# laboroai/border

Measured on AMD Instinct MI355X. Metric: agent opt-steps/sec (DQN Atari 84x84x4, batch 256), higher is better.
Workload: dtype f32 (conv2 / conv3 forward: 3xbf16 operand split, 6 products)

## Files before the change

border_amd/csrc/conv1_dw_bf16.hpp:

```cpp
#pragma once
#include "conv1_bf16.hpp"

namespace bdr {

struct Conv1DwArgs {
    const uint8_t* x;
    const float* dy;
    float* part;
    size_t part_stride;
    int B;
};

constexpr int C1DW_LDM = 408;
constexpr int C1DW_ROW = 88, C1DW_CH = 84 * 88 + 96;
#ifndef C1DW_WAVES_PER_EU
#define C1DW_WAVES_PER_EU 3
#endif
constexpr int C1DW_PF = 2;

struct __attribute__((packed, aligned(4))) U32x4A4 { uint32_t x, y, z, w; };

template <int PH>
__device__ __forceinline__ uint32_t u8pair_to_bf16(uint32_t d0, uint32_t d1)
{
    const uint32_t f0 = __float_as_uint((float)((d0 >> (8 * PH)) & 255u)), f1 = __float_as_uint((float)((d1 >> (8 * PH)) & 255u));
    return __builtin_amdgcn_perm(f1, f0, 0x07060302u);
}

#ifdef C1DW_TRACE
__device__ unsigned long long* g_c1dw_trace;
#define C1DW_TP(slot) do { if (threadIdx.x == 0 && g_c1dw_trace) g_c1dw_trace[blockIdx.x * 4 + (slot)] = wall_clock64(); } while (0)
#else
#define C1DW_TP(slot) do { } while (0)
#endif

__device__ __forceinline__ void c1dw_load_step(const uint8_t* src, int s, int g, U32x4A4 (&d)[2])
{
#pragma unroll
    for (int q = 0; q < 2; ++q) {
        const int quad = 2 * s + q;
        const int oh = quad / 5, ow0 = 4 * (quad - 5 * oh);
        const uint32_t* p = reinterpret_cast<const uint32_t*>(src + (4 * oh) * C1DW_ROW + 4 * ow0);
        d[q].x = p[0]; d[q].y = p[1]; d[q].z = p[2]; d[q].w = p[3];
    }
}

template <int PH, int TPW>
__device__ __forceinline__ void c1dw_steps(const uint8_t* const (&src)[TPW], U32x4A4 (&ring)[TPW][C1DW_PF + 1][2], const uint16_t* planes, int i, int g,
                                           f32x16 (&acc)[TPW])
{
    uint4 bq[3], bn[3];
#pragma unroll
    for (int pl = 0; pl < 3; ++pl) bq[pl] = *reinterpret_cast<const uint4*>(&planes[(pl * 32 + i) * C1DW_LDM + 200 * g]);
#pragma unroll
    for (int s = 0; s < 25; ++s) {
        if (s + 1 < 25) {
#pragma unroll
            for (int pl = 0; pl < 3; ++pl) bn[pl] = *reinterpret_cast<const uint4*>(&planes[(pl * 32 + i) * C1DW_LDM + 8 * (s + 1) + 200 * g]);
        }
#pragma unroll
        for (int t = 0; t < TPW; ++t) {
            U32x4A4 (&cur)[2] = ring[t][s % (C1DW_PF + 1)];
            if (s + C1DW_PF < 25) c1dw_load_step(src[t], s + C1DW_PF, g, ring[t][(s + C1DW_PF) % (C1DW_PF + 1)]);
            uint4 av;
            av.x = u8pair_to_bf16<PH>(cur[0].x, cur[0].y);
            av.y = u8pair_to_bf16<PH>(cur[0].z, cur[0].w);
            av.z = u8pair_to_bf16<PH>(cur[1].x, cur[1].y);
            av.w = u8pair_to_bf16<PH>(cur[1].z, cur[1].w);
            const bf16x8 af = __builtin_bit_cast(bf16x8, av);
#pragma unroll
            for (int pl = 2; pl >= 0; --pl)
                acc[t] = __builtin_amdgcn_mfma_f32_32x32x16_bf16(af, __builtin_bit_cast(bf16x8, bq[pl]), acc[t], 0, 0, 0);
        }
#pragma unroll
        for (int pl = 0; pl < 3; ++pl) bq[pl] = bn[pl];
        __builtin_amdgcn_sched_barrier(0);
    }
}

template <int NS>
static __global__ __launch_bounds__(512) __attribute__((amdgpu_waves_per_eu(NS <= 4 ? C1DW_WAVES_PER_EU : 2, NS <= 4 ? C1DW_WAVES_PER_EU : 2))) void k_conv1_dw_bf16(Conv1DwArgs a)
{
    C1DW_TP(0);
    constexpr int TASKS = 4 * ((NS + 1) / 2), TPW = (TASKS + 7) / 8;
    extern __shared__ __attribute__((aligned(16))) uint8_t c1dw_lds[];
    uint16_t* planes = reinterpret_cast<uint16_t*>(c1dw_lds);
    uint32_t* ximg_l = reinterpret_cast<uint32_t*>(c1dw_lds + 3 * 32 * C1DW_LDM * 2);
    float (*sred)[32] = reinterpret_cast<float (*)[32]>(c1dw_lds + 3 * 32 * C1DW_LDM * 2 + NS * C1DW_CH);
    const int tid = threadIdx.x, lane = tid & 63, wave = __builtin_amdgcn_readfirstlane(tid >> 6);
    const int i = lane & 31, g = lane >> 5;
    const int pn = tid & 31, pmg = tid >> 5;
    const int phase = wave & 3;

    f32x16 acc[TPW];
#pragma unroll
    for (int t = 0; t < TPW; ++t)
#pragma unroll
        for (int r = 0; r < 16; ++r) acc[t][r] = 0.f;
    float bsum = 0.f;

    int c_of[TPW], rowoff; bool live[TPW];
    rowoff = ((i >> 1) & 7) * C1DW_ROW + 4 * (i & 1) + g * (40 * C1DW_ROW);
#pragma unroll
    for (int t = 0; t < TPW; ++t) {
        const int task = wave + 8 * t;
        live[t] = task < TASKS;
        const int c = 2 * ((live[t] ? task : 0) >> 2) + (i >> 4);
        c_of[t] = c < NS ? c : NS - 1;
    }

    for (int img = blockIdx.x; img < a.B; img += gridDim.x) {
        constexpr int XPT = (NS * 441 + 511) / 512;
        uint4 xst[XPT];
        {
            const uint4* xg = reinterpret_cast<const uint4*>(a.x + (size_t)img * (NS * 7056));
#pragma unroll
            for (int k = 0; k < XPT; ++k) { const int t = tid + 512 * k; xst[k] = xg[t < NS * 441 ? t : NS * 441 - 1]; }
        }
        {
            const float* dyb = a.dy + (size_t)img * 400 * 32;
            float s = 0.f;
#pragma unroll
            for (int q0 = 0; q0 < 7; q0 += 4) {
                float y[4][4];
#pragma unroll
                for (int q = 0; q < 4; ++q) {
                    const int quad = pmg + 16 * (q0 + q);
#pragma unroll
                    for (int j = 0; j < 4; ++j) y[q][j] = (q0 + q < 7 && quad < 100) ? dyb[(size_t)(4 * quad + j) * 32 + pn] : 0.f;
                }
#pragma unroll
                for (int q = 0; q < 4; ++q) {
                    const int quad = pmg + 16 * (q0 + q);
                    if (q0 + q < 7 && quad < 100) {
                        uint32_t hi[4], mid[4], lo[4];
#pragma unroll
                        for (int j = 0; j < 4; ++j) {
                            s += y[q][j];
                            hi[j] = __float_as_uint(y[q][j]) & 0xffff0000u;
                            const float r1 = y[q][j] - __uint_as_float(hi[j]);
                            mid[j] = __float_as_uint(r1) & 0xffff0000u;
                            const float r2 = r1 - __uint_as_float(mid[j]);
                            lo[j] = __float_as_uint(r2) & 0xffff0000u;
                        }
                        const int o = pn * C1DW_LDM + 4 * quad;
                        *reinterpret_cast<uint2*>(&planes[0 * 32 * C1DW_LDM + o]) = uint2{(hi[0] >> 16) | hi[1], (hi[2] >> 16) | hi[3]};
                        *reinterpret_cast<uint2*>(&planes[1 * 32 * C1DW_LDM + o]) = uint2{(mid[0] >> 16) | mid[1], (mid[2] >> 16) | mid[3]};
                        *reinterpret_cast<uint2*>(&planes[2 * 32 * C1DW_LDM + o]) = uint2{(lo[0] >> 16) | lo[1], (lo[2] >> 16) | lo[3]};
                    }
                }
            }
            sred[pmg][pn] = s;
        }
#pragma unroll
        for (int k = 0; k < XPT; ++k) {
            const int t = tid + 512 * k;
            if (t < NS * 441) {
                const uint32_t w[4] = {xst[k].x, xst[k].y, xst[k].z, xst[k].w};
#pragma unroll
                for (int e = 0; e < 4; ++e) {
                    const int d = 4 * t + e, c = d / 1764, rem = d - c * 1764, r = rem / 21;
                    ximg_l[c * (C1DW_CH / 4) + r * (C1DW_ROW / 4) + (rem - r * 21)] = w[e];
                }
            }
        }
        __syncthreads();
        C1DW_TP(1);
        if (tid < 32) {
            float t = sred[0][tid];
#pragma unroll
            for (int k = 1; k < 16; ++k) t += sred[k][tid];
            bsum += t;
        }

        const uint8_t* src[TPW];
        U32x4A4 ring[TPW][C1DW_PF + 1][2];
#pragma unroll
        for (int t = 0; t < TPW; ++t) {
            src[t] = reinterpret_cast<const uint8_t*>(ximg_l) + c_of[t] * C1DW_CH + rowoff;
#pragma unroll
            for (int s0 = 0; s0 < C1DW_PF; ++s0) c1dw_load_step(src[t], s0, g, ring[t][s0]);
        }
        if (live[0]) {
            if (phase == 0) c1dw_steps<0, TPW>(src, ring, planes, i, g, acc);
            else if (phase == 1) c1dw_steps<1, TPW>(src, ring, planes, i, g, acc);
            else if (phase == 2) c1dw_steps<2, TPW>(src, ring, planes, i, g, acc);
            else c1dw_steps<3, TPW>(src, ring, planes, i, g, acc);
        }
        C1DW_TP(2);
        __syncthreads();
    }

    float* part = a.part + (size_t)blockIdx.x * a.part_stride;
#pragma unroll
    for (int t = 0; t < TPW; ++t) {
        if (!live[t]) continue;
        const int pair = (wave + 8 * t) >> 2;
#pragma unroll
        for (int r = 0; r < 16; ++r) {
            const int row = (r & 3) + 8 * (r >> 2) + 4 * g;
            const int c = 2 * pair + (row >> 4), kh = (row >> 1) & 7, kw = phase + 4 * (row & 1);
            if (c < NS) part[(size_t)(c * 64 + kh * 8 + kw) * 32 + i] = acc[t][r];
        }
    }
    if (tid < 32) part[64 * NS * 32 + tid] = bsum;
    C1DW_TP(3);
}

constexpr size_t c1dw_lds_bytes(int ns) { return (size_t)3 * 32 * C1DW_LDM * 2 + (size_t)ns * C1DW_CH + 16 * 32 * 4; }

inline hipError_t launch_conv1_dw_bf16(int ns, dim3 grid, hipStream_t st, const Conv1DwArgs& d)
{
    switch (ns) {
#define BDR_C1DW_CASE(N) case N: { \
            static bool allowed[64] = {false};    \
            int dev = 0; \
            if (hipGetDevice(&dev) != hipSuccess || dev < 0 || dev >= 64) return hipErrorInvalidDevice; \
            if (!allowed[dev]) { \
                const hipError_t e = hipFuncSetAttribute(reinterpret_cast<const void*>(&k_conv1_dw_bf16<N>), hipFuncAttributeMaxDynamicSharedMemorySize, (int)c1dw_lds_bytes(N)); \
                if (e != hipSuccess) return e; \
                allowed[dev] = true; \
            } \
            hipLaunchKernelGGL(k_conv1_dw_bf16<N>, grid, dim3(512), c1dw_lds_bytes(N), st, d); break; }
        BDR_C1DW_CASE(1) BDR_C1DW_CASE(2) BDR_C1DW_CASE(3) BDR_C1DW_CASE(4) BDR_C1DW_CASE(5) BDR_C1DW_CASE(6) BDR_C1DW_CASE(7) BDR_C1DW_CASE(8)
#undef BDR_C1DW_CASE
        default: return hipErrorInvalidValue;
    }
    return hipGetLastError();
}

}
```

border_amd/csrc/dqn.hip:

```cpp
#include <algorithm>
#include <atomic>
#include <chrono>
#include <cmath>
#include <string>

#include "common.hpp"
#include "agent_base.hpp"
#include "igemm.hpp"
#include "conv1_bf16_img.hpp"
#include "cnn_layers.hpp"
#include "igemm_b3.hpp"
#include "act_small.hpp"

using namespace bdr;

namespace {

#ifndef BDR_TEAMS
#define BDR_TEAMS 2
#endif
#ifndef BDR_TEAMS_FWD_C3
#define BDR_TEAMS_FWD_C3 BDR_TEAMS
#endif
#ifndef BDR_TEAMS_DX_L1
#define BDR_TEAMS_DX_L1 BDR_TEAMS
#endif
#ifndef BDR_TEAMS_DX_C3
#define BDR_TEAMS_DX_C3 BDR_TEAMS
#endif
#ifndef BDR_TEAMS_FWD_L1
#define BDR_TEAMS_FWD_L1 1
#endif
#ifndef BDR_TEAMS_FWD_C2
#define BDR_TEAMS_FWD_C2 1
#endif
#ifndef BDR_TEAMS_DX_C2
#define BDR_TEAMS_DX_C2 1
#endif
#ifndef BDR_DXC2_MERGED
#define BDR_DXC2_MERGED 2
#endif
#ifndef BDR_FWDC3_SHAPE
#define BDR_FWDC3_SHAPE 1, 2, 1, 1
#endif
using FwdC3D = FwdConvP<GeomC3, BDR_FWDC3_SHAPE>;
constexpr size_t PL2_U16 = (size_t)3 * 64 * 512, PL3_U16 = (size_t)3 * 64 * 576;
constexpr size_t CPL_W2 = 0, CPL_W3 = PL2_U16, CPL_U16 = PL2_U16 + PL3_U16;
__device__ __forceinline__ size_t cpl_index(int k, int n) { return ((size_t)(k >> 5) * 64 + n) * 32 + (k & 31); }

__device__ __forceinline__ void conv_plane_store(uint16_t* __restrict__ pl, int layer, int e, float x)
{
    uint16_t v[3];
    split3_rn(x, v);
    const size_t n = (size_t)(layer ? 576 : 512) * 64, o = cpl_index(e >> 6, e & 63);
    uint16_t* d = pl + (layer ? CPL_W3 : CPL_W2);
    d[o] = v[0]; d[n + o] = v[1]; d[2 * n + o] = v[2];
}

__global__ __launch_bounds__(256) void k_conv_planes(const float* __restrict__ w2, const float* __restrict__ w3, uint16_t* __restrict__ pl)
{
    const int i = blockIdx.x * 256 + threadIdx.x;
    if (i < 512 * 64) conv_plane_store(pl, 0, i, w2[i]);
    else if (i < 512 * 64 + 576 * 64) conv_plane_store(pl, 1, i - 512 * 64, w3[i - 512 * 64]);
}
#ifndef BDR_FWDC2_B3_SHAPE
#define BDR_FWDC2_B3_SHAPE 2, 2
#endif
#ifndef BDR_FWDC3_B3_SHAPE
#define BDR_FWDC3_B3_SHAPE 2, 2
#endif
struct FwdB3Args : FwdArgs { const uint16_t* wpl[MAXZ]; };
template <class G, int WM_, int WN_, int TM_ = 1, int TN_ = 1>
struct FwdB3 : FwdP<G, AFwd<G>, WM_, WN_, false, 0, TM_, TN_> {
    using Args = FwdB3Args;
    __device__ static const uint4* b_chunk(const Args& a, int z, int, int pl, int kt, int n, int kq)
    {
        return reinterpret_cast<const uint4*>(a.wpl[z] + (size_t)pl * G::COUT * G::K + cpl_index(kt * 32 + kq * 8, n));
    }
};
using FwdC2B3 = FwdB3<GeomC2, BDR_FWDC2_B3_SHAPE>;
using FwdC3B3 = FwdB3<GeomC3, BDR_FWDC3_B3_SHAPE>;
constexpr int TEAMS_FWD_C2 = BDR_TEAMS_FWD_C2, TEAMS_FWD_C3 = BDR_TEAMS_FWD_C3, TEAMS_FWD_L1 = BDR_TEAMS_FWD_L1, TEAMS_DX_L1 = BDR_TEAMS_DX_L1,
              TEAMS_DX_C3 = BDR_TEAMS_DX_C3, TEAMS_DX_C2 = BDR_TEAMS_DX_C2;

struct HeadArgs {
    const float* p1[MAXZ];
    const float* b4[MAXZ];
    const float* w5[MAXZ];
    const float* b5[MAXZ];
    float* h1[MAXZ];
    float* q[MAXZ];
    int B, A, S;
};

struct TdArgs {
    int double_dqn;
    const uint8_t* act;
    int act_bytes;
    const float* reward;
    const int8_t* term;
    float* dh1;
    float* dq;
    float* pred;
    float* tgt;
    float* loss_row;
    int B, A;
    float gamma;
    int loss_kind;
    const float* weight;
    float* td_abs;
    int has_clip; float clip_min, clip_max;
    unsigned* err;
    const float* q_tgt_mem;
    int z_tgt, z_sel;
    unsigned* wait_sig; unsigned wait_epoch; unsigned long long wait_limit; unsigned* sig_err;
};

constexpr int HEAD_ROWS = 2;
template <int S, int AMAX>
__global__ __launch_bounds__(64 * HEAD_ROWS * MAXZ) void k_head(HeadArgs a, TdArgs t, int nz, int td)
{
    __shared__ float sq[HEAD_ROWS][MAXZ][64];
    const int lane = threadIdx.x & 63, wave = __builtin_amdgcn_readfirstlane(threadIdx.x >> 6);
    const int r = wave / nz, z = wave % nz;
    const int row = blockIdx.x * HEAD_ROWS + r;
    const bool valid = row < a.B;
    const int rw = valid ? row : 0;
    const int A = a.A;
    f32x4 part[S][2];
#pragma unroll
    for (int s = 0; s < S; ++s) {
        const float* p = a.p1[z] + ((size_t)s * a.B + rw) * 512 + lane * 8;
        part[s][0] = *reinterpret_cast<const f32x4*>(p);
        part[s][1] = *reinterpret_cast<const f32x4*>(p + 4);
    }
    const f32x4 b4lo = *reinterpret_cast<const f32x4*>(a.b4[z] + lane * 8), b4hi = *reinterpret_cast<const f32x4*>(a.b4[z] + lane * 8 + 4);
    const float* w5 = a.w5[z] + lane * 8;
    float wreg[8][AMAX];
#pragma unroll
    for (int k = 0; k < AMAX; ++k) {
        const float* wk = w5 + (size_t)min(k, A - 1) * 512;
        const f32x4 lo = *reinterpret_cast<const f32x4*>(wk), hi = *reinterpret_cast<const f32x4*>(wk + 4);
#pragma unroll
        for (int j = 0; j < 4; ++j) { wreg[j][k] = lo[j]; wreg[4 + j][k] = hi[j]; }
    }
    const float b5 = lane < A ? a.b5[z][lane] : 0.f;
    long long act = 0; float reward = 0.f, wgt = 1.f; int term = 0;
    if (td && z == 0) {
        act = *reinterpret_cast<const long long*>(t.act + (size_t)rw * t.act_bytes);
        if (act < 0 || act >= A) {
            if (lane == 0 && t.err) atomicOr(t.err + bdr_agent::ERR_ACTION, 1u);
            act = act < 0 ? 0 : A - 1;
        }
        reward = t.reward[rw]; term = (int)t.term[rw];
        if (t.weight) wgt = t.weight[rw];
    }

    f32x4 h[2] = {f32x4{0, 0, 0, 0}, f32x4{0, 0, 0, 0}};
#pragma unroll
    for (int s = 0; s < S; ++s) { h[0] += part[s][0]; h[1] += part[s][1]; }
    float hv[8];
#pragma unroll
    for (int j = 0; j < 8; ++j) {
        const float v = h[j >> 2][j & 3] + (j < 4 ? b4lo[j & 3] : b4hi[j & 3]);
        hv[j] = v > 0.f ? v : 0.f;
    }
    asm volatile("" ::"v"(act), "v"(reward), "v"(term), "v"(wgt), "v"(b5));
    if (valid) {
        float* ho = a.h1[z] + (size_t)row * 512 + lane * 8;
        *reinterpret_cast<f32x4*>(ho) = f32x4{hv[0], hv[1], hv[2], hv[3]};
        *reinterpret_cast<f32x4*>(ho + 4) = f32x4{hv[4], hv[5], hv[6], hv[7]};
    }
    float sk[AMAX];
#pragma unroll
    for (int k = 0; k < AMAX; ++k) {
        float s = 0.f;
#pragma unroll
        for (int j = 0; j < 8; ++j) s = fmaf(hv[j], wreg[j][k], s);
        sk[k] = s;
    }
#pragma unroll
    for (int off = 32; off > 0; off >>= 1)
#pragma unroll
        for (int k = 0; k < AMAX; ++k) sk[k] += __shfl_xor(sk[k], off);
    float qv = 0.f;
#pragma unroll
    for (int k = 0; k < AMAX; ++k) qv = lane == k ? sk[k] : qv;
    qv += b5;
    if (lane < A) {
        if (valid) a.q[z][(size_t)row * A + lane] = qv;
        sq[r][z][lane] = qv;
    }
    if (!td) return;
    if (t.q_tgt_mem && t.wait_sig) {
        if (threadIdx.x == 0) {
            const unsigned long long t0 = wall_clock64();
            while ((int)(__hip_atomic_load(t.wait_sig, __ATOMIC_ACQUIRE, __HIP_MEMORY_SCOPE_AGENT) - t.wait_epoch) < 0) {
                __builtin_amdgcn_s_sleep(2);
                if (__hip_atomic_load(t.sig_err, __ATOMIC_RELAXED, __HIP_MEMORY_SCOPE_AGENT) != 0) break;
                if (wall_clock64() - t0 > t.wait_limit) {
                    __hip_atomic_store(t.sig_err, 100u, __ATOMIC_RELAXED, __HIP_MEMORY_SCOPE_AGENT);
                    if (t.err) __hip_atomic_store(t.err + bdr_agent::ERR_GATE, 100u, __ATOMIC_RELAXED, __HIP_MEMORY_SCOPE_AGENT);
                    break;
                }
            }
        }
    }
    __syncthreads();
    if (z != 0 || !valid) return;
    if (t.q_tgt_mem) {
        __builtin_amdgcn_fence(__ATOMIC_ACQUIRE, "agent");
        if (lane < A) sq[r][MAXZ - 1][lane] = __builtin_nontemporal_load(t.q_tgt_mem + (size_t)row * A + lane);
    }
    const float* q_tg = t.q_tgt_mem ? sq[r][MAXZ - 1] : sq[r][t.z_tgt];
    const float* sel = t.z_sel >= 0 ? sq[r][t.z_sel] : q_tg;
    float v = lane < A ? sel[lane] : -INFINITY;
    int idx = lane;
#pragma unroll
    for (int off = 32; off > 0; off >>= 1) {
        const float ov = __shfl_xor(v, off);
        const int oi = __shfl_xor(idx, off);
        if (ov > v || (ov == v && oi < idx)) { v = ov; idx = oi; }
    }
    const float qn = q_tg[idx];
    const float pred = sq[r][0][act];
    const float tgt = td_target(reward, (float)(1 - term), t.gamma, qn);
    const TdLossIn li{t.loss_kind, t.weight != nullptr, wgt, t.has_clip, t.clip_min, t.clip_max};
    float lossb, tdv;
    const float dl = td_loss_row(pred, tgt, li, lossb, tdv);
    const float dq = dl / (float)a.B;
    if (lane == 0) {
        t.dq[row] = dq; t.pred[row] = pred; t.tgt[row] = tgt; t.loss_row[row] = lossb;
        if (t.td_abs) t.td_abs[row] = tdv;
    }
    float out[8];
#pragma unroll
    for (int j = 0; j < 8; ++j) {
        float wj = 0.f;
#pragma unroll
        for (int k = 0; k < AMAX; ++k) wj = (int)act == k ? wreg[j][k] : wj;
        out[j] = hv[j] > 0.f ? dq * wj : 0.f;
    }
    float* o = t.dh1 + (size_t)row * 512 + lane * 8;
    *reinterpret_cast<f32x4*>(o) = f32x4{out[0], out[1], out[2], out[3]};
    *reinterpret_cast<f32x4*>(o + 4) = f32x4{out[4], out[5], out[6], out[7]};
}

struct HeadBwdArgs {
    const float* h1; const float* dq; const uint8_t* act; int act_bytes;
    const float* loss_row;
    float* gw5; float* gb5; float* loss;
    int B, A;
};
__global__ __launch_bounds__(256) void k_head_bwd(HeadBwdArgs a)
{
    __shared__ int s_rows[256];
    __shared__ float s_dq[256];
    __shared__ int s_wcnt[4];
    __shared__ float s_red[256];
    const int tid = threadIdx.x, lane = tid & 63, wave = tid >> 6;
    if ((int)blockIdx.x == 2 * a.A) {
        float s = 0.f;
        for (int b = tid; b < a.B; b += 256) s += a.loss_row[b];
        s_red[tid] = s;
        __syncthreads();
        for (int w = 128; w > 0; w >>= 1) {
            if (tid < w) s_red[tid] += s_red[tid + w];
            __syncthreads();
        }
        if (tid == 0) a.loss[0] = s_red[0] / (float)a.B;
        return;
    }
    const int ac = blockIdx.x >> 1, j = (blockIdx.x & 1) * 256 + tid;
    float acc = 0.f, bacc = 0.f;
    for (int b0 = 0; b0 < a.B; b0 += 256) {
        const int b = b0 + tid;
        bool match = false;
        float dqv = 0.f;
        if (b < a.B) {
            match = *reinterpret_cast<const long long*>(a.act + (size_t)b * a.act_bytes) == ac;
            dqv = a.dq[b];
        }
        const unsigned long long m = __ballot(match);
        if (lane == 0) s_wcnt[wave] = __popcll(m);
        __syncthreads();
        int base = 0;
        for (int w = 0; w < wave; ++w) base += s_wcnt[w];
        const int total = s_wcnt[0] + s_wcnt[1] + s_wcnt[2] + s_wcnt[3], padded = (total + 15) & ~15;
        if (match) {
            const int pos = base + __popcll(m & ((1ull << lane) - 1ull));
            s_rows[pos] = b; s_dq[pos] = dqv;
        }
        if (tid >= total && tid < padded) { s_rows[tid] = b0; s_dq[tid] = 0.f; }
        __syncthreads();
        for (int k = 0; k < padded; k += 16) {
            float hvv[16];
#pragma unroll
            for (int u = 0; u < 16; ++u) hvv[u] = a.h1[(size_t)s_rows[k + u] * 512 + j];
            if (k == 0 && tid == 0) for (int q = 0; q < total; ++q) bacc += s_dq[q];
#pragma unroll
            for (int u = 0; u < 16; ++u) acc = fmaf(k + u < total ? hvv[u] : 0.f, s_dq[k + u], acc);
        }
        __syncthreads();
    }
    a.gw5[(size_t)ac * 512 + j] = acc;
    if (tid == 0 && (blockIdx.x & 1) == 0) a.gb5[ac] = bacc;
}

}

struct DqnCnn : bdr_agent {
    bdr_dqn_config cfg;
    hipStream_t side = nullptr;
    hipStream_t aux = nullptr;
    hipEvent_t ev_fork[4] = {nullptr}, ev_join = nullptr;
    bool kev = true;
    unsigned* sig = nullptr;
    unsigned sig_epoch = 0;
    unsigned test_epoch = 0;
    bool aux_gated = true;
    bool head_gate_enqueued = false;
    bool side_gather = true;
    unsigned long long* gate_trace = nullptr;
    int sched = 3;
    unsigned long long gate_limit = 1000000000ull;
    bool holds_gate_token = false;
    bool defer_adam = false;
    bool split_fwd = true;
    bool noted_event_fallback = false;
    bool three_queues = true;
    bool tgt_enqueued = false;
    unsigned track_epoch = 0;
    bool track_wait_pending = false;
    hipStream_t comm_st = nullptr;
    int comm_state = 0;
    unsigned xchg_epoch = 0;
    bool xchg_pending_conv = false, xchg_pending_fc = false, xchg_tracked = false;
    Arena ar;
    int B = 0;
    float *q = nullptr, *q_tgt = nullptr, *grad = nullptr, *m = nullptr, *v = nullptr;
    float* vmax = nullptr; bool amsgrad = false;
    float* a1[MAXZ] = {nullptr}; float* a2[MAXZ] = {nullptr}; float* a3[MAXZ] = {nullptr};
    float* p1[MAXZ] = {nullptr}; float* h1[MAXZ] = {nullptr}; float* qv[MAXZ] = {nullptr};
    float *dh1 = nullptr, *dy3 = nullptr, *dy2 = nullptr, *dy1 = nullptr;
    float *dq = nullptr, *pred = nullptr, *tgt = nullptr, *loss_row = nullptr, *loss = nullptr;
    float *part = nullptr; size_t part_floats = 0;
    uint8_t *u_obs = nullptr, *u_next = nullptr, *u_act = nullptr; float* u_rew = nullptr; int8_t* u_term = nullptr;
    uint64_t u_cap = 0;
    const float* last_reward = nullptr; int last_B = 0;
    uint64_t adam_step = 0, soft_update_counter = 0;
    int64_t conv_step_lag = 0;
    uint16_t* cpl[2] = {nullptr, nullptr};
    bool cpl_fresh[2] = {false, false}, cpl_escaped[2] = {false, false};
    bool conv_b3 = true;
    void planes_stale(int set) { if (set == 0 || set == 1) cpl_fresh[set] = false; }
    void arena_escaped(int which) override { if (which == 0 || which == 1) cpl_escaped[which] = true; }
    void arena_released(int which) override { if (which == 0 || which == 1) { cpl_escaped[which] = false; cpl_fresh[which] = false; } }
    float* act_part = nullptr; unsigned* act_tickets = nullptr;
    unsigned long long* applied_step = nullptr;

    ~DqnCnn() override;
    const char* kind() const override { return "dqn_cnn"; }
    int32_t opt(bdr_replay* r) override;
    void on_gate_timeout() override;
    void drain_queues() override
    {
        (void)hipStreamSynchronize(stream);
        if (side) (void)hipStreamSynchronize(side);
        if (aux) (void)hipStreamSynchronize(aux);
        if (comm_st) (void)hipStreamSynchronize(comm_st);
    }
    int32_t after_sync() override
    {
        if (!(xchg_pending_conv || xchg_pending_fc)) return BDR_OK;
        BDR_TRY(join_exchange(true, true));
        BDR_HIP(hipStreamSynchronize(stream));
        return BDR_OK;
    }
    int32_t grads_on_batch(uint64_t n, const void* obs, const int64_t* act, const void* next_obs, const float* reward, const int8_t* term) override;
    int32_t apply_grads() override;
    int exchange_plan(int which, ExchangeSeg* segs, int cap, hipStream_t* comm) override;
    int32_t exchange_begin(int seg) override;
    int32_t exchange_end(int seg) override;
    int32_t join_exchange(bool conv, bool fc);
    int32_t record(float* out, int cap, int* n) override;
    void record_keys(std::vector<std::string>& keys) override;
    uint64_t param_count(int which) override;
    int32_t get_params(int which, float* out, uint64_t n) override;
    int32_t set_params(int which, const float* in, uint64_t n) override;
    float* arena(int which, size_t* n) override;
    int32_t save(const char* dir) override;
    int32_t load(const char* dir) override;
};

namespace {


void free_batch_buffers(DqnCnn* a)
{
    for (int z = 0; z < MAXZ; ++z) {
        (void)hipFree(a->a1[z]); (void)hipFree(a->a2[z]); (void)hipFree(a->a3[z]);
        (void)hipFree(a->p1[z]); (void)hipFree(a->h1[z]); (void)hipFree(a->qv[z]);
        a->a1[z] = a->a2[z] = a->a3[z] = a->p1[z] = a->h1[z] = a->qv[z] = nullptr;
    }
    (void)hipFree(a->dh1); (void)hipFree(a->dy3); (void)hipFree(a->dy2); (void)hipFree(a->dy1);
    (void)hipFree(a->dq); (void)hipFree(a->pred); (void)hipFree(a->tgt); (void)hipFree(a->loss_row);
    (void)hipFree(a->part);
    a->dh1 = a->dy3 = a->dy2 = a->dy1 = a->dq = a->pred = a->tgt = a->loss_row = a->part = nullptr;
}

int32_t ensure_batch(DqnCnn* a, int B)
{
    if (B <= a->B) return BDR_OK;
    BDR_HIP(hipStreamSynchronize(a->stream));
    free_batch_buffers(a);
    const int A = a->ar.A;
    for (int z = 0; z < MAXZ; ++z) {
        BDR_TRY(alloc_f(&a->a1[z], (size_t)B * 400 * 32));
        BDR_TRY(alloc_f(&a->a2[z], (size_t)B * 81 * 64));
        BDR_TRY(alloc_f(&a->a3[z], (size_t)B * 49 * 64));
        BDR_TRY(alloc_f(&a->p1[z], (size_t)L1_SPLIT * B * 512));
        BDR_TRY(alloc_f(&a->h1[z], (size_t)B * 512));
        BDR_TRY(alloc_f(&a->qv[z], (size_t)B * A));
    }
    BDR_TRY(alloc_f(&a->dh1, (size_t)B * 512));
    BDR_TRY(alloc_f(&a->dy3, (size_t)B * 49 * 64));
    BDR_TRY(alloc_f(&a->dy2, (size_t)B * 81 * 64));
    BDR_TRY(alloc_f(&a->dy1, (size_t)B * 400 * 32));
    BDR_TRY(alloc_f(&a->dq, B)); BDR_TRY(alloc_f(&a->pred, B)); BDR_TRY(alloc_f(&a->tgt, B));
    BDR_TRY(alloc_f(&a->loss_row, B));
    const DwPlan p = dw_plan(B, a->ar.ns);
    BDR_TRY(alloc_f(&a->part, p.total));
    a->part_floats = p.total;
    a->B = B;
    return BDR_OK;
}

struct ConvReduceAdamArgs {
    Reduce3Args r;
    float* p; const float* g; float* m; float* v;
    float* gbase;
    size_t rest0_4, n4;
    AdamScalars s;
    int reduce_blocks;
    const unsigned* poison;
    int reduce_only;
    unsigned long long* applied; unsigned long long step;
    uint16_t* cpl;
};
constexpr int SIG_HEAD = 0, SIG_DXL1 = 1, SIG_DXC3 = 2, SIG_SIDE = 3, SIG_GATHER = 4, SIG_TEST = 5, SIG_TEST_ERR = 6, SIG_ERR = 7, SIG_TGT = 8, SIG_TRACK = 9, SIG_MAIN_END = 10, SIG_XCONV = 11, SIG_XFC = 14;
__global__ __launch_bounds__(64) void k_gate(unsigned* sig, int which, unsigned epoch, unsigned long long* waited, int publish,
                                             unsigned long long limit = 1000000000ull , int err_slot = SIG_ERR,
                                             unsigned* dev_err = nullptr)
{
    if (threadIdx.x != 0) return;
    if (publish >= 0) __hip_atomic_store(sig + publish, epoch, __ATOMIC_RELAXED, __HIP_MEMORY_SCOPE_AGENT);
    if (err_slot == SIG_ERR && __hip_atomic_load(sig + SIG_ERR, __ATOMIC_RELAXED, __HIP_MEMORY_SCOPE_AGENT) != 0) return;
    const unsigned long long t0 = wall_clock64();
    while ((int)(__hip_atomic_load(sig + which, __ATOMIC_ACQUIRE, __HIP_MEMORY_SCOPE_AGENT) - epoch) < 0) {
        __builtin_amdgcn_s_sleep(4);
        if (wall_clock64() - t0 > limit || (err_slot == SIG_ERR && __hip_atomic_load(sig + SIG_ERR, __ATOMIC_RELAXED, __HIP_MEMORY_SCOPE_AGENT) != 0)) {
            __hip_atomic_store(sig + err_slot, 1u + (unsigned)which, __ATOMIC_RELAXED, __HIP_MEMORY_SCOPE_AGENT);
            if (dev_err) __hip_atomic_store(dev_err + bdr_agent::ERR_GATE, 1u + (unsigned)which, __ATOMIC_RELAXED, __HIP_MEMORY_SCOPE_AGENT);
            return;
        }
    }
    if (waited) {
        const unsigned long long dt = wall_clock64() - t0;
        waited[0] += dt; waited[1] += 1;
        unsigned long long* mx = waited + 22 - (which == SIG_SIDE ? 4 : which);
        if (dt > *mx) *mx = dt;
        if (which == SIG_SIDE) {
            const unsigned long long ts = *reinterpret_cast<volatile unsigned long long*>(sig + 12);
            if (ts && t0 > ts) waited[12] += t0 - ts;
        }
    }
}
__global__ __launch_bounds__(64) void k_signal(unsigned* sig, int which, unsigned epoch)
{
    if (threadIdx.x == 0 && which == SIG_SIDE) *reinterpret_cast<volatile unsigned long long*>(sig + 12) = wall_clock64();
    if (threadIdx.x == 0) __hip_atomic_store(sig + which, epoch, __ATOMIC_RELAXED, __HIP_MEMORY_SCOPE_AGENT);
}

__global__ void k_copy_word_unless(unsigned long long* dst, const unsigned long long* src, const unsigned* poison) { if (!(poison && *poison)) *dst = *src; }

__global__ __launch_bounds__(256) void k_reduce_adam(ConvReduceAdamArgs a)
{
    const bool poisoned = a.reduce_only || (a.poison && *a.poison != 0);
    if (a.applied && !poisoned && blockIdx.x == 0 && threadIdx.x == 0) *a.applied = a.step;
    if ((int)blockIdx.x >= a.reduce_blocks) {
        if (poisoned) return;
        const size_t i = a.rest0_4 + (size_t)(blockIdx.x - a.reduce_blocks) * 256 + threadIdx.x;
        if (i >= a.n4) return;
        f32x4 pp = reinterpret_cast<f32x4*>(a.p)[i], gg = reinterpret_cast<const f32x4*>(a.g)[i];
        f32x4 mm = reinterpret_cast<f32x4*>(a.m)[i], vv = reinterpret_cast<f32x4*>(a.v)[i];
#pragma unroll
        for (int j = 0; j < 4; ++j) {
            float pe = pp[j], me = mm[j], ve = vv[j];
            adam_element(pe, gg[j], me, ve, a.s);
            pp[j] = pe; mm[j] = me; vv[j] = ve;
        }
        reinterpret_cast<f32x4*>(a.p)[i] = pp;
        reinterpret_cast<f32x4*>(a.m)[i] = mm;
        reinterpret_cast<f32x4*>(a.v)[i] = vv;
        return;
    }
    __shared__ float red[8][32];
    const int s_id = (int)blockIdx.x >= a.r.seg[2].wg0 ? 2 : ((int)blockIdx.x >= a.r.seg[1].wg0 ? 1 : 0);
    const ReduceSeg& sg = a.r.seg[s_id];
    const int o = threadIdx.x & 31, grp = threadIdx.x >> 5;
    const int i = ((int)blockIdx.x - sg.wg0) * 32 + o;
    float s = 0.f;
    if (i < sg.n) {
        int c = grp;
        for (; c + 24 < sg.chunks; c += 32) {
            const float v0 = sg.part[(size_t)c * sg.stride + i], v1 = sg.part[(size_t)(c + 8) * sg.stride + i];
            const float v2 = sg.part[(size_t)(c + 16) * sg.stride + i], v3 = sg.part[(size_t)(c + 24) * sg.stride + i];
            s += v0; s += v1; s += v2; s += v3;
        }
        for (; c < sg.chunks; c += 8) s += sg.part[(size_t)c * sg.stride + i];
    }
    red[grp][o] = s;
    __syncthreads();
    if (grp == 0 && i < sg.n) {
        float t = red[0][o];
#pragma unroll
        for (int k = 1; k < 8; ++k) t += red[k][o];
        const float g = i < sg.n_weights ? t * sg.wscale : t;
        sg.g[i] = g;
        if (poisoned) return;
        const size_t e = (size_t)(sg.g - a.gbase) + i;
        float pe = a.p[e], me = a.m[e], ve = a.v[e];
        adam_element(pe, g, me, ve, a.s);
        a.p[e] = pe; a.m[e] = me; a.v[e] = ve;
        if (a.cpl && s_id >= 1 && i < sg.n_weights) conv_plane_store(a.cpl, s_id - 1, i, pe);
    }
}

int effective_sched(DqnCnn* a);

struct NetInst { const uint8_t* x; const float* params; int slot; };

int32_t forward(DqnCnn* a, const NetInst* inst, int nz, int B, const TdArgs* td = nullptr, hipStream_t st = nullptr)
{
    if (!st) st = a->stream;
    const Arena& ar = a->ar;
    FwdArgs f{};
    bool uses_q = false;
    for (int z = 0; z < nz; ++z) uses_q = uses_q || inst[z].params == a->q;
    if (uses_q) BDR_TRY(a->join_exchange(true, false));
    {
        Conv1Args c{};
        c.M = B * 400; c.nz = nz;
        for (int z = 0; z < nz; ++z) {
            c.x[z] = inst[z].x; c.w1[z] = inst[z].params + ar.w1; c.bias[z] = inst[z].params + ar.b1; c.out[z] = a->a1[inst[z].slot];
        }
        Bracket br(a, "fwd_conv1");
        BDR_HIP(conv1_forward(ar.ns, B, st, c));
    }
    f.M = B * 81;
    for (int z = 0; z < nz; ++z) { f.x[z] = a->a1[inst[z].slot]; f.w[z] = inst[z].params + ar.w2; f.bias[z] = inst[z].params + ar.b2; f.out[z] = a->a2[inst[z].slot]; }
    bool b3 = a->conv_b3;
    FwdB3Args fb{};
    for (int z = 0; z < nz && b3; ++z) b3 = inst[z].params == a->q || inst[z].params == a->q_tgt;
    for (int z = 0; z < nz && b3; ++z) {
        const int set = inst[z].params == a->q ? 0 : 1;
        if (a->cpl_fresh[set] && !a->cpl_escaped[set]) continue;
        hipLaunchKernelGGL(k_conv_planes, dim3((512 * 64 + 576 * 64 + 255) / 256), dim3(256), 0, st, inst[z].params + ar.w2, inst[z].params + ar.w3, a->cpl[set]);
        BDR_HIP(hipGetLastError());
        a->cpl_fresh[set] = true;
    }
    if (b3) {
        static_cast<FwdArgs&>(fb) = f;
        for (int z = 0; z < nz; ++z) fb.wpl[z] = a->cpl[inst[z].params == a->q ? 0 : 1] + CPL_W2;
        Bracket br(a, "fwd_conv2");
        BDR_HIP((launch_igemm_b3<FwdC2B3, 6>(st, dim3(m_tiles<FwdC2B3>(f.M) * n_tiles<FwdC2B3>(), 1, nz), fb)));
    } else { Bracket br(a, "fwd_conv2"); BDR_HIP((launch_igemm<FwdC2, TEAMS_FWD_C2>(st, dim3(m_tiles<FwdC2>(f.M) * n_tiles<FwdC2>(), 1, nz), f))); }
    f.M = B * 49;
    for (int z = 0; z < nz; ++z) { f.x[z] = a->a2[inst[z].slot]; f.w[z] = inst[z].params + ar.w3; f.bias[z] = inst[z].params + ar.b3; f.out[z] = a->a3[inst[z].slot]; }
    if (b3) {
        static_cast<FwdArgs&>(fb) = f;
        for (int z = 0; z < nz; ++z) fb.wpl[z] = a->cpl[inst[z].params == a->q ? 0 : 1] + CPL_W3;
        Bracket br(a, "fwd_conv3");
        BDR_HIP((launch_igemm_b3<FwdC3B3, 6>(st, dim3(m_tiles<FwdC3B3>(f.M) * n_tiles<FwdC3B3>(), 1, nz), fb)));
    } else { Bracket br(a, "fwd_conv3"); BDR_HIP((launch_igemm<FwdC3D, TEAMS_FWD_C3>(st, dim3(m_tiles<FwdC3D>(f.M) * n_tiles<FwdC3D>(), 1, nz), f))); }
    f.M = B; f.nkt_per_split = (98 + L1_SPLIT - 1) / L1_SPLIT;
    for (int z = 0; z < nz; ++z) { f.x[z] = a->a3[inst[z].slot]; f.w[z] = inst[z].params + ar.w4; f.bias[z] = nullptr; f.out[z] = a->p1[inst[z].slot]; }
    if (uses_q) BDR_TRY(a->join_exchange(false, true));
    {
        Bracket br(a, "fwd_l1");
#if BDR_L1_XSPLIT
        static_assert(L1_SPLIT == 8, "FwdL1X: one k-slice per XCD");
        BDR_HIP((launch_igemm<FwdL1X, TEAMS_FWD_L1>(st, dim3(m_tiles<FwdL1X>(B) * n_tiles<FwdL1X>() * 8, 1, nz), f)));
#else
        if (nz % 2 == 0) BDR_HIP((launch_igemm<FwdL1Z2, TEAMS_FWD_L1>(st, dim3(((B + 63) / 64) * 16, L1_SPLIT, nz / 2), f)));
        else BDR_HIP((launch_igemm<FwdL1, TEAMS_FWD_L1>(st, dim3(((B + 63) / 64) * 8, L1_SPLIT, nz), f)));
#endif
    }
    HeadArgs h{};
    h.B = B; h.A = ar.A; h.S = L1_SPLIT;
    for (int z = 0; z < nz; ++z) {
        h.p1[z] = a->p1[inst[z].slot]; h.b4[z] = inst[z].params + ar.b4; h.w5[z] = inst[z].params + ar.w5;
        h.b5[z] = inst[z].params + ar.b5; h.h1[z] = a->h1[inst[z].slot]; h.q[z] = a->qv[inst[z].slot];
    }
    {
        Bracket br(a, td ? "head_fwd_td" : "head_fwd");
        const dim3 grid((B + HEAD_ROWS - 1) / HEAD_ROWS), block(64 * HEAD_ROWS * nz);
        const TdArgs tv = td ? *td : TdArgs{};
        hipEvent_t stop = td && effective_sched(a) == 1 && a->kev ? a->ev_fork[0] : nullptr;
        const int tdi = td ? 1 : 0;
        if (ar.A <= 8) hipExtLaunchKernelGGL((k_head<L1_SPLIT, 8>), grid, block, 0, st, nullptr, stop, 0, h, tv, nz, tdi);
        else if (ar.A <= 24) hipExtLaunchKernelGGL((k_head<L1_SPLIT, 24>), grid, block, 0, st, nullptr, stop, 0, h, tv, nz, tdi);
        else hipExtLaunchKernelGGL((k_head<L1_SPLIT, 64>), grid, block, 0, st, nullptr, stop, 0, h, tv, nz, tdi);
        BDR_HIP(hipGetLastError());
    }
    return BDR_OK;
}

AdamScalars adam_scalars(const bdr_dqn_config& c, uint64_t step)
{
    return adam_scalars_for(c.opt_kind == BDR_OPT_ADAMW, c.lr, c.beta1, c.beta2, c.eps, c.weight_decay, step);
}

int32_t launch_gate(DqnCnn* a, hipStream_t st, int which, unsigned epoch, int publish)
{
    unsigned long long* tr = a->gate_trace && which <= SIG_SIDE ? a->gate_trace + 2 * (st == a->stream ? 4 : which) : nullptr;
    hipLaunchKernelGGL(k_gate, dim3(1), dim3(64), 0, st, a->sig, which, epoch, tr, publish, a->gate_limit, SIG_ERR, a->dev_err);
    BDR_HIP(hipGetLastError());
    return BDR_OK;
}

int32_t queues_independent(DqnCnn* a, hipStream_t waiter, hipStream_t producer, bool* ok)
{
    a->test_epoch += 1;
    BDR_HIP(hipMemsetAsync(a->sig + SIG_TEST_ERR, 0, sizeof(unsigned), waiter));
    hipLaunchKernelGGL(k_gate, dim3(1), dim3(64), 0, waiter, a->sig, SIG_TEST, a->test_epoch, (unsigned long long*)nullptr, -1, 10000000ull, SIG_TEST_ERR,
                       (unsigned*)nullptr);
    BDR_HIP(hipGetLastError());
    hipLaunchKernelGGL(k_signal, dim3(1), dim3(64), 0, producer, a->sig, SIG_TEST, a->test_epoch);
    BDR_HIP(hipGetLastError());
    BDR_HIP(hipStreamSynchronize(waiter));
    BDR_HIP(hipStreamSynchronize(producer));
    unsigned err = 0;
    BDR_HIP(hipMemcpy(&err, a->sig + SIG_TEST_ERR, sizeof err, hipMemcpyDeviceToHost));
    *ok = err == 0;
    return BDR_OK;
}

std::atomic<DqnCnn*> g_gate_owner{nullptr};
bool claim_gates(DqnCnn* a)
{
    if (a->holds_gate_token) return true;
    DqnCnn* expected = nullptr;
    if (g_gate_owner.compare_exchange_strong(expected, a)) { a->holds_gate_token = true; return true; }
    return false;
}
int effective_sched(DqnCnn* a)
{
    if (a->prof) return 0;
    if (a->sched == 3 && !claim_gates(a)) {
        if (!a->noted_event_fallback) {
            a->noted_event_fallback = true;
            fprintf(stderr, "border_amd: another DQN agent of this process already orders its two queues with device flags; this agent orders its "
                            "queues with events (same results, ~10 %% slower steps) for as long as that agent lives\n");
        }
        return 1;
    }
    return a->sched;
}

int32_t update_critic(DqnCnn* a, int B, const uint8_t* obs, const uint8_t* next_obs, const uint8_t* act, int act_bytes,
                      const float* reward, const int8_t* term, const float* weight = nullptr, bdr_replay* per_buffer = nullptr)
{
    BDR_TRY(ensure_batch(a, B));
    BDR_TRY(a->td_buffer(B));
    a->last_reward = reward; a->last_B = B;
    const Arena& ar = a->ar;
    const bdr_dqn_config& c = a->cfg;
    NetInst inst[3] = {{obs, a->q, 0}, {next_obs, a->q_tgt, 1}, {next_obs, a->q, 2}};

    TdArgs t{};
    t.double_dqn = c.double_dqn;
    t.act = act; t.act_bytes = act_bytes; t.reward = reward; t.term = term;
    t.dh1 = a->dh1; t.dq = a->dq; t.pred = a->pred; t.tgt = a->tgt;
    t.loss_row = a->loss_row; t.B = B; t.A = ar.A; t.gamma = (float)c.discount_factor; t.loss_kind = c.critic_loss;
    t.weight = weight; t.td_abs = a->td_abs;
    t.has_clip = c.has_clip_td_err; t.clip_min = (float)c.clip_td_err_min; t.clip_max = (float)c.clip_td_err_max;
    t.err = a->dev_err;
    t.z_tgt = 1; t.z_sel = c.double_dqn ? 2 : -1;
    if (a->tgt_enqueued) {
        a->tgt_enqueued = false;
        NetInst on[2] = {{obs, a->q, 0}, {next_obs, a->q, 2}};
        t.q_tgt_mem = a->qv[1]; t.z_tgt = -1; t.z_sel = c.double_dqn ? 1 : -1;
        t.wait_sig = a->sig + SIG_TGT; t.wait_epoch = a->sig_epoch + 1; t.wait_limit = a->gate_limit; t.sig_err = a->sig + SIG_ERR;
        BDR_TRY(forward(a, on, c.double_dqn ? 2 : 1, B, &t));
    } else {
        BDR_TRY(forward(a, inst, c.double_dqn ? 3 : 2, B, &t));
    }

    const int sched = effective_sched(a);
    const bool ov = sched == 1;
    const bool gated = sched == 3;
    hipStream_t sd = ov || gated ? a->side : a->stream;
    const unsigned epoch = gated ? ++a->sig_epoch : 0;
    auto sigf = [&](int which) -> unsigned* { return gated ? a->sig + which : nullptr; };
    auto gate = [&](hipStream_t st, int which) -> int32_t { return launch_gate(a, st, which, epoch, -1); };
    const unsigned any = sched == 2 ? hipExtAnyOrderLaunch : 0;
    auto kev = [&](int k) -> hipEvent_t { return ov && a->kev ? a->ev_fork[k] : nullptr; };
    auto fork = [&](int k) -> int32_t {
        if (!ov) return BDR_OK;
        if (!a->kev) BDR_HIP(hipEventRecord(a->ev_fork[k], a->stream));
        BDR_HIP(hipStreamWaitEvent(a->side, a->ev_fork[k], 0));
        return BDR_OK;
    };
    const DwPlan pl = dw_plan(a->B, ar.ns);
    const bool defer = a->defer_adam;
    if (!defer) a->adam_step += 1;
    const AdamScalars adam_s = adam_scalars(c, std::max<uint64_t>(a->adam_step, 1));

    auto head_bwd = [&]() -> int32_t {
        HeadBwdArgs hb{a->h1[0], a->dq, act, act_bytes, a->loss_row, a->grad + ar.w5, a->grad + ar.b5, a->loss, B, ar.A};
        Bracket br(a, "head_bwd");
        LAUNCH_FL(sd, any, nullptr, k_head_bwd, dim3(2 * ar.A + 1), dim3(256), hb);
        return BDR_OK;
    };
    auto l1_dw = [&]() -> int32_t {
        DwArgs d{a->a3[0], a->dh1, a->grad + ar.w4, 0, B};
        Bracket br(a, "bwd_l1_dw");
        LAUNCH_FL(sd, any, nullptr, k_igemm_red<DwL1>, dim3(49 * 8), dim3(256), d);
        return BDR_OK;
    };
    auto l1_dx = [&]() -> int32_t {
        DxArgs d{a->dh1, a->q + ar.w4, a->a3[0], a->dy3, B, sigf(SIG_HEAD), epoch};
        Bracket br(a, "bwd_l1_dx");
        BDR_HIP((launch_igemm<DxL1, TEAMS_DX_L1>(a->stream, dim3((m_tiles<DxL1>(B) * n_tiles<DxL1>() + 7) / 8 * 8, 1, 1), d, 0, kev(1))));
        return BDR_OK;
    };
    auto adam_l1_l2 = [&]() -> int32_t {
        if (defer) return BDR_OK;
        Bracket br(a, "adam_l1_l2");
        const size_t r4 = (ar.total - ar.w4) / 4;
        LAUNCH_FL(sd, any, nullptr, k_adam, dim3((unsigned)((r4 + 255) / 256)), dim3(256), a->q + ar.w4, (const float*)(a->grad + ar.w4), a->m + ar.w4,
                  a->v + ar.w4, r4, adam_s, (const unsigned*)(a->sig + SIG_ERR), a->applied_step, (unsigned long long)a->adam_step);
        return BDR_OK;
    };
    auto c3_dw = [&]() -> int32_t {
        const int M = B * 49, chunks = std::min(pl.chunks_c3, (M + 31) / 32);
        DwArgs d{a->a2[0], a->dy3, a->part + pl.off_c3, pl.stride_c3, M};
        Bracket br(a, "bwd_conv3_dw");
        LAUNCH_FL(sd, any, nullptr, k_igemm_red<DwC3>, dim3(9 * chunks), dim3(256), d);
        return BDR_OK;
    };
    auto c3_dx = [&]() -> int32_t {
        DxArgs d{a->dy3, a->q + ar.w3, a->a2[0], a->dy2, B * 81, sigf(SIG_DXL1), epoch};
        Bracket br(a, "bwd_conv3_dx");
        BDR_HIP((launch_igemm<DxC3Pos, TEAMS_DX_C3>(a->stream, dim3(((B + DxC3Pos::WM * DxC3Pos::TM * 32 - 1) / (DxC3Pos::WM * DxC3Pos::TM * 32)) * n_tiles<DxC3Pos>(), 81, 1), d, 0, kev(2))));
        return BDR_OK;
    };
    auto c2_dw = [&]() -> int32_t {
        const int M = B * 81, chunks = std::min(pl.chunks_c2, (M + 31) / 32);
        DwArgs d{a->a1[0], a->dy2, a->part + pl.off_c2, pl.stride_c2, M, nullptr, 0};
        Bracket br(a, "bwd_conv2_dw");
        LAUNCH_FL(sd, any, ov && a->kev ? a->ev_join : nullptr, k_igemm_red<DwC2>, dim3(8 * chunks), dim3(256), d);
        return BDR_OK;
    };
    auto c2_dx = [&]() -> int32_t {
        DxArgs d{a->dy2, a->q + ar.w2, a->a1[0], a->dy1, B * 100, sigf(SIG_DXC3), epoch};
        Bracket br(a, "bwd_conv2_dx");
#if BDR_DXC2_MERGED == 2
        BDR_HIP((launch_igemm<DxC2MPos, TEAMS_DX_C2>(a->stream, dxc2_pos_grid<DxC2MPos>(B), d)));
#elif BDR_DXC2_MERGED
        BDR_HIP((launch_igemm<DxC2M, TEAMS_DX_C2>(a->stream, dim3(m_tiles<DxC2M>(d.M) * n_tiles<DxC2M>(), 1, 1), d)));
#else
        BDR_HIP((launch_igemm<DxC2, TEAMS_DX_C2>(a->stream, dim3((d.M + 127) / 128, 4, 1), d)));
#endif
        return BDR_OK;
    };
    auto c1_dw = [&]() -> int32_t {
        const int chunks = std::min(pl.chunks_c1, B);
        Conv1DwArgs d{obs, a->dy1, a->part + pl.off_c1, pl.stride_c1, B};
        Bracket br(a, "bwd_conv1_dw");
        BDR_HIP(launch_conv1_dw_bf16(ar.ns, dim3(chunks), a->stream, d));
        return BDR_OK;
    };

    const bool per = per_buffer && weight;
    if (per && sched == 2) BDR_HIP(hipEventRecord(a->ev_fork[0], a->stream));
    BDR_TRY(fork(0));
    if (per) {
        hipStream_t ps = a->stream;
        if (sched != 0) {
            if (gated && a->aux_gated) BDR_TRY(gate(a->aux, SIG_HEAD));
            else {
                if (gated) BDR_HIP(hipEventRecord(a->ev_fork[0], a->stream));
                BDR_HIP(hipStreamWaitEvent(a->aux, a->ev_fork[0], 0));
            }
            ps = a->aux;
        }
        Bracket br(a, "per_update");
        BDR_TRY(replay_update_priority_on_stream(per_buffer, B, a->td_abs, ps));
    }
    if (gated) {
        if (!a->head_gate_enqueued) BDR_TRY(gate(sd, SIG_HEAD));
        a->head_gate_enqueued = false;
        BDR_TRY(head_bwd()); BDR_TRY(l1_dw());
        BDR_TRY(l1_dx());
        BDR_TRY(gate(sd, SIG_DXL1)); BDR_TRY(c3_dw()); BDR_TRY(adam_l1_l2());
        hipLaunchKernelGGL(k_signal, dim3(1), dim3(64), 0, sd, a->sig, SIG_SIDE, epoch);
        BDR_HIP(hipGetLastError());
        BDR_TRY(c3_dx());
        BDR_TRY(c2_dx());
        { hipStream_t side = sd; sd = a->stream; BDR_TRY(c2_dw()); sd = side; }
        BDR_TRY(c1_dw());
        BDR_TRY(gate(a->stream, SIG_SIDE));
    } else if (sched == 2) {
        BDR_TRY(l1_dx());  BDR_TRY(head_bwd()); BDR_TRY(l1_dw());
        BDR_TRY(c3_dx());  BDR_TRY(adam_l1_l2()); BDR_TRY(c3_dw());
        BDR_TRY(c2_dx());  BDR_TRY(c2_dw());
        BDR_TRY(c1_dw());
    } else {
        BDR_TRY(head_bwd()); BDR_TRY(l1_dw());
        BDR_TRY(l1_dx());
        BDR_TRY(fork(1));
        BDR_TRY(adam_l1_l2()); BDR_TRY(c3_dw());
        BDR_TRY(c3_dx());
        BDR_TRY(fork(2));
        BDR_TRY(c2_dw());
        BDR_TRY(c2_dx());
        BDR_TRY(c1_dw());
        if (ov) {
            if (!a->kev) BDR_HIP(hipEventRecord(a->ev_join, a->side));
            BDR_HIP(hipStreamWaitEvent(a->stream, a->ev_join, 0));
        }
    }
    {
        Reduce3Args r{};
        const int Ms[3] = {B * 400, B * 81, B * 49};
        const int plc[3] = {pl.chunks_c1, pl.chunks_c2, pl.chunks_c3};
        const size_t offs[3] = {pl.off_c1, pl.off_c2, pl.off_c3}, strides[3] = {pl.stride_c1, pl.stride_c2, pl.stride_c3};
        const size_t gw[3] = {ar.w1, ar.w2, ar.w3};
        const int nw[3] = {(int)ar.n_w1(), 512 * 64, 576 * 64}, nb[3] = {32, 64, 64};
        int wg = 0;
        for (int k = 0; k < 3; ++k) {
            const int nchunks = k == 0 ? std::min(plc[0], B) : std::min(plc[k], (Ms[k] + 31) / 32);
            r.seg[k] = ReduceSeg{a->part + offs[k], strides[k], nchunks, a->grad + gw[k], nw[k] + nb[k], nw[k],
                                 k == 0 ? INV255 : 1.0f, wg};
            wg += (nw[k] + nb[k] + 31) / 32;
        }
        ConvReduceAdamArgs ra{};
        ra.r = r; ra.p = a->q; ra.g = a->grad; ra.m = a->m; ra.v = a->v; ra.gbase = a->grad;
        ra.rest0_4 = ra.n4 = ar.w4 / 4; ra.s = a->conv_step_lag ? adam_scalars(c, (uint64_t)std::max<int64_t>((int64_t)a->adam_step - a->conv_step_lag, 1)) : adam_s;
        ra.applied = defer ? nullptr : a->applied_step + 1; ra.step = (unsigned long long)((int64_t)a->adam_step - a->conv_step_lag);
        ra.reduce_blocks = wg; ra.poison = a->sig + SIG_ERR; ra.reduce_only = defer ? 1 : 0;
        ra.cpl = a->conv_b3 && !defer ? a->cpl[0] : nullptr;
        Bracket br(a, "reduce_adam");
        hipLaunchKernelGGL(k_reduce_adam, dim3(wg), dim3(256), 0, a->stream, ra);
        BDR_HIP(hipGetLastError());
        if (ra.cpl) a->cpl_fresh[0] = true;
    }
    return BDR_OK;
}

int32_t soft_update(DqnCnn* a)
{
    const size_t n4 = a->ar.total / 4;
    const float tau = (float)a->cfg.tau, omt = (float)(1.0 - a->cfg.tau);
    Bracket br(a, "track");
    a->planes_stale(1);
    hipLaunchKernelGGL(k_track, dim3((unsigned)((n4 + 255) / 256)), dim3(256), 0, a->stream, a->q_tgt, a->q, n4, tau, omt, (const unsigned*)(a->sig + SIG_ERR));
    BDR_HIP(hipGetLastError());
    if (a->sig_epoch != 0 && a->split_fwd && !a->prof) {
        a->track_epoch = a->sig_epoch;
        hipLaunchKernelGGL(k_signal, dim3(1), dim3(64), 0, a->stream, a->sig, SIG_TRACK, a->track_epoch);
        BDR_HIP(hipGetLastError());
        a->track_wait_pending = true;
    }
    return BDR_OK;
}

int32_t after_updates(DqnCnn* a)
{
    a->soft_update_counter += 1;
    if (a->soft_update_counter == a->cfg.soft_update_interval) {
        a->soft_update_counter = 0;
        BDR_TRY(soft_update(a));
    }
    a->n_opts += 1;
    return BDR_OK;
}

int32_t adam_all(DqnCnn* a)
{
    a->adam_step += 1;
    a->planes_stale(0);
    Bracket br(a, "adam_all");
    const size_t n4 = a->ar.total / 4;
    const unsigned* poison = (const unsigned*)(a->sig + SIG_ERR);
    struct Range { size_t off, n; uint64_t step; int slot; } rg[2] = {{0, a->ar.total, a->adam_step, 0}, {0, 0, 0, 1}};
    int nr = 1;
    if (a->conv_step_lag) {
        const uint64_t cs = (uint64_t)std::max<int64_t>((int64_t)a->adam_step - a->conv_step_lag, 1);
        rg[0] = Range{a->ar.w4, a->ar.total - a->ar.w4, a->adam_step, 0}; rg[1] = Range{0, a->ar.w4, cs, 1}; nr = 2;
    }
    for (int k = 0; k < nr; ++k) {
        const Range& g = rg[k];
        const AdamScalars sc = adam_scalars(a->cfg, g.step);
        if (a->amsgrad) { BDR_TRY(launch_adam_amsgrad(a->stream, a->q + g.off, a->grad + g.off, a->m + g.off, a->v + g.off, a->vmax + g.off, g.n, sc, poison, a->applied_step + g.slot, (unsigned long long)g.step)); continue; }
        hipLaunchKernelGGL(k_adam, dim3((unsigned)((g.n / 4 + 255) / 256)), dim3(256), 0, a->stream, a->q + g.off, (const float*)(a->grad + g.off), a->m + g.off, a->v + g.off, g.n / 4,
                           sc, poison, a->applied_step + g.slot, (unsigned long long)g.step);
        BDR_HIP(hipGetLastError());
    }
    if (nr == 1) {
        hipLaunchKernelGGL(k_copy_word_unless, dim3(1), dim3(1), 0, a->stream, a->applied_step + 1, (const unsigned long long*)a->applied_step, poison);
        BDR_HIP(hipGetLastError());
    }
    (void)n4;
    return BDR_OK;
}

int32_t opt_inner(DqnCnn* a, bdr_replay* r)
{
    BDR_REQUIRE(r->obs_bytes == (uint64_t)a->cfg.net.n_stack * 84 * 84, "replay obs rows (%llu B) do not match the AtariCnn input",
                (unsigned long long)r->obs_bytes);
    BDR_REQUIRE(r->act_bytes >= 8, "discrete actions are stored as i64");
    BDR_REQUIRE(r->device == a->device, "agent and replay buffer live on different devices");
    { Bracket br(a, "_null"); }
    BDR_TRY(ensure_batch(a, (int)a->cfg.batch_size));
    BDR_TRY(a->td_buffer(a->cfg.batch_size));
    for (uint64_t u = 0; u < a->cfg.n_updates_per_opt; ++u) {
        if (effective_sched(a) == 3 && a->side_gather) {
            const unsigned epoch = a->sig_epoch + 1;
            BDR_TRY(replay_flip_batch(r, a->cfg.batch_size));
            const bool tq3 = a->split_fwd && a->three_queues && !r->per && a->aux_gated;
            hipStream_t tq = tq3 ? a->aux : a->side;
            if (tq3) BDR_TRY(launch_gate(a, tq, SIG_HEAD, epoch - 1, -1));
            BDR_TRY(replay_sample_on_stream(r, a->cfg.batch_size, tq));
            if (a->split_fwd) {
                hipLaunchKernelGGL(k_signal, dim3(1), dim3(64), 0, tq, a->sig, SIG_GATHER, epoch);
                BDR_HIP(hipGetLastError());
                if (a->track_wait_pending) {
                    BDR_TRY(launch_gate(a, tq, SIG_TRACK, a->track_epoch, -1));
                    a->track_wait_pending = false;
                }
                NetInst tg[1] = {{r->b_next, a->q_tgt, 1}};
                BDR_TRY(forward(a, tg, 1, (int)a->cfg.batch_size, nullptr, tq));
                if (tq3) {
                    hipLaunchKernelGGL(k_signal, dim3(1), dim3(64), 0, tq, a->sig, SIG_TGT, epoch);
                    BDR_HIP(hipGetLastError());
                    BDR_TRY(launch_gate(a, a->side, SIG_HEAD, epoch, -1));
                } else {
                    BDR_TRY(launch_gate(a, a->side, SIG_HEAD, epoch, SIG_TGT));
                }
                a->tgt_enqueued = true;
            } else {
                BDR_TRY(launch_gate(a, a->side, SIG_HEAD, epoch, SIG_GATHER));
            }
            a->head_gate_enqueued = true;
            BDR_TRY(launch_gate(a, a->stream, SIG_GATHER, epoch, -1));
        } else {
            Bracket br(a, "sample");
            BDR_TRY(replay_sample_on_stream(r, a->cfg.batch_size, a->stream));
        }
        a->defer_adam = a->grad_comm != nullptr || a->amsgrad;
        const int32_t st = update_critic(a, (int)a->cfg.batch_size, r->b_obs, r->b_next, r->b_act, (int)r->act_bytes, r->b_reward, r->b_term,
                                         replay_batch_weights(r), r);
        a->defer_adam = false;
        BDR_TRY(st);
        if (a->grad_comm) {
            Bracket br(a, "grad_allreduce"); BDR_TRY(a->grad_reduce(a, a->grad_comm));
        }
        if (a->grad_comm || a->amsgrad) BDR_TRY(adam_all(a));
    }
    return after_updates(a);
}

int32_t fill_record(DqnCnn* a, int B, const float* reward_dev, bdr_dqn_record* rec)
{
    BDR_HIP(hipMemcpyAsync(&rec->loss, a->loss, 4, hipMemcpyDeviceToHost, a->stream));
    BDR_HIP(hipStreamSynchronize(a->stream));
    rec->has_verbose = 0;
    if (a->cfg.record_verbose_level >= 2) {
        std::vector<float> p(B), t(B), rw(B);
        BDR_HIP(hipMemcpy(p.data(), a->pred, B * 4, hipMemcpyDeviceToHost));
        BDR_HIP(hipMemcpy(t.data(), a->tgt, B * 4, hipMemcpyDeviceToHost));
        BDR_HIP(hipMemcpy(rw.data(), reward_dev, B * 4, hipMemcpyDeviceToHost));
        double sp = 0, st = 0, sr = 0, sd = 0;
        for (int i = 0; i < B; ++i) { sp += p[i]; st += t[i]; sr += rw[i]; sd += (double)t[i] - p[i]; }
        rec->pred_mean = (float)(sp / B); rec->tgt_mean = (float)(st / B); rec->reward_mean = (float)(sr / B);
        rec->tgt_minus_pred_mean = (float)(sd / B);
        rec->has_verbose = 1;
    }
    return BDR_OK;
}

size_t ref_param_count(int A, int ns) { return (size_t)2048 * ns + 32 + 32768 + 64 + 36864 + 64 + (size_t)512 * 3136 + 512 + (size_t)A * 512 + A; }

void to_internal(const Arena& ar, const float* ref, float* in)
{
    std::fill(in, in + ar.total, 0.f);
    const float* p = ref;
    const int K1 = 64 * ar.ns;
    for (int o = 0; o < 32; ++o) for (int k = 0; k < K1; ++k) in[ar.w1 + (size_t)k * 32 + o] = p[(size_t)o * K1 + k];
    p += (size_t)32 * K1; std::copy(p, p + 32, in + ar.b1); p += 32;
    for (int o = 0; o < 64; ++o) for (int c = 0; c < 32; ++c) for (int kh = 0; kh < 4; ++kh) for (int kw = 0; kw < 4; ++kw)
        in[ar.w2 + (size_t)((kh * 4 + kw) * 32 + c) * 64 + o] = p[((size_t)(o * 32 + c) * 4 + kh) * 4 + kw];
    p += 32768; std::copy(p, p + 64, in + ar.b2); p += 64;
    for (int o = 0; o < 64; ++o) for (int c = 0; c < 64; ++c) for (int kh = 0; kh < 3; ++kh) for (int kw = 0; kw < 3; ++kw)
        in[ar.w3 + (size_t)((kh * 3 + kw) * 64 + c) * 64 + o] = p[((size_t)(o * 64 + c) * 3 + kh) * 3 + kw];
    p += 36864; std::copy(p, p + 64, in + ar.b3); p += 64;
    for (int o = 0; o < 512; ++o) for (int c = 0; c < 64; ++c) for (int hw = 0; hw < 49; ++hw)
        in[ar.w4 + (size_t)(hw * 64 + c) * 512 + o] = p[(size_t)o * 3136 + c * 49 + hw];
    p += (size_t)512 * 3136; std::copy(p, p + 512, in + ar.b4); p += 512;
    std::copy(p, p + (size_t)ar.A * 512, in + ar.w5);
    p += (size_t)ar.A * 512; std::copy(p, p + ar.A, in + ar.b5);
}

void to_reference(const Arena& ar, const float* in, float* ref)
{
    float* p = ref;
    const int K1 = 64 * ar.ns;
    for (int o = 0; o < 32; ++o) for (int k = 0; k < K1; ++k) p[(size_t)o * K1 + k] = in[ar.w1 + (size_t)k * 32 + o];
    p += (size_t)32 * K1; std::copy(in + ar.b1, in + ar.b1 + 32, p); p += 32;
    for (int o = 0; o < 64; ++o) for (int c = 0; c < 32; ++c) for (int kh = 0; kh < 4; ++kh) for (int kw = 0; kw < 4; ++kw)
        p[((size_t)(o * 32 + c) * 4 + kh) * 4 + kw] = in[ar.w2 + (size_t)((kh * 4 + kw) * 32 + c) * 64 + o];
    p += 32768; std::copy(in + ar.b2, in + ar.b2 + 64, p); p += 64;
    for (int o = 0; o < 64; ++o) for (int c = 0; c < 64; ++c) for (int kh = 0; kh < 3; ++kh) for (int kw = 0; kw < 3; ++kw)
        p[((size_t)(o * 64 + c) * 3 + kh) * 3 + kw] = in[ar.w3 + (size_t)((kh * 3 + kw) * 64 + c) * 64 + o];
    p += 36864; std::copy(in + ar.b3, in + ar.b3 + 64, p); p += 64;
    for (int o = 0; o < 512; ++o) for (int c = 0; c < 64; ++c) for (int hw = 0; hw < 49; ++hw)
        p[(size_t)o * 3136 + c * 49 + hw] = in[ar.w4 + (size_t)(hw * 64 + c) * 512 + o];
    p += (size_t)512 * 3136; std::copy(in + ar.b4, in + ar.b4 + 512, p); p += 512;
    std::copy(in + ar.w5, in + ar.w5 + (size_t)ar.A * 512, p);
    p += (size_t)ar.A * 512; std::copy(in + ar.b5, in + ar.b5 + ar.A, p);
}

float* arena_ptr(DqnCnn* a, int which)
{
    switch (which) {
        case 0: return a->q; case 1: return a->q_tgt; case 2: return a->m; case 3: return a->v; case 4: return a->grad;
        case 5: return a->vmax;
        default: return nullptr;
    }
}

void init_reference_params(int A, int ns, uint64_t seed, std::vector<float>& ref)
{
    ref.resize(ref_param_count(A, ns));
    const size_t sizes[10] = {(size_t)2048 * ns, 32, 32768, 64, 36864, 64, (size_t)512 * 3136, 512, (size_t)A * 512, (size_t)A};
    const int fan[10] = {64 * ns, 64 * ns, 512, 512, 576, 576, 3136, 3136, 512, 512};
    uint64_t s = seed * 0x9E3779B97F4A7C15ull + 0x1234567ull;
    size_t o = 0;
    for (int t = 0; t < 10; ++t) {
        const float bound = 1.0f / std::sqrt((float)fan[t]);
        for (size_t i = 0; i < sizes[t]; ++i) {
            s += 0x9E3779B97F4A7C15ull;
            uint64_t x = s; x ^= x >> 30; x *= 0xBF58476D1CE4E5B9ull; x ^= x >> 27; x *= 0x94D049BB133111EBull; x ^= x >> 31;
            ref[o + i] = ((float)(x >> 40) * (2.0f / 16777216.0f) - 1.0f) * bound;
        }
        o += sizes[t];
    }
}

}


void DqnCnn::on_gate_timeout()
{
    (void)hipStreamSynchronize(stream);
    if (side) (void)hipStreamSynchronize(side);
    if (aux) (void)hipStreamSynchronize(aux);
    if (comm_st) (void)hipStreamSynchronize(comm_st);
    xchg_pending_conv = xchg_pending_fc = false;
    planes_stale(0); planes_stale(1);
    if (sig) (void)hipMemset(sig, 0, 16 * sizeof(unsigned));
    if (applied_step) {
        unsigned long long applied[2] = {0, 0};
        if (hipMemcpy(applied, applied_step, sizeof applied, hipMemcpyDeviceToHost) == hipSuccess) {
            const int64_t conv_now = (int64_t)adam_step - conv_step_lag;
            if (applied[0] < adam_step || (int64_t)applied[1] < conv_now) {
                const uint64_t skipped = adam_step - std::min<uint64_t>(applied[0], adam_step);
                adam_step -= skipped;
                conv_step_lag = (int64_t)adam_step - (int64_t)std::min<uint64_t>(applied[1], (uint64_t)std::max<int64_t>(conv_now, 0));
                const uint64_t opts_back = std::min(n_opts, skipped / std::max<uint64_t>(1, cfg.n_updates_per_opt));
                n_opts -= opts_back;
                const uint64_t iv = std::max<uint64_t>(1, cfg.soft_update_interval);
                soft_update_counter = (soft_update_counter + iv - opts_back % iv) % iv;
                fprintf(stderr, "border_amd: %llu update(s) behind the failed gate were skipped on the device; the step counters were rolled back with them%s\n",
                        (unsigned long long)skipped, conv_step_lag ? " (the conv segment is one optimizer step behind l1 / l2 and keeps its own step number)" : "");
            }
        }
    }
    sig_epoch = 0; head_gate_enqueued = false;
    if (sched == 3) {
        fprintf(stderr, "border_amd: a cross-queue gate timed out; this agent continues with event ordering (schedule 1)\n");
        sched = 1;
    }
    if (holds_gate_token) { DqnCnn* me = this; g_gate_owner.compare_exchange_strong(me, nullptr); holds_gate_token = false; }
}

int DqnCnn::exchange_plan(int which, ExchangeSeg* segs, int cap, hipStream_t* comm)
{
    if (which != 0 || cap < 2 || sig_epoch == 0 || getenv("BDR_NO_XCHG_OVERLAP")) return 0;
    if (effective_sched(this) != 3 || xchg_pending_conv || xchg_pending_fc) return 0;
    if (comm_state == 0) {
        comm_state = -1;
        if (hipStreamCreateWithFlags(&comm_st, hipStreamNonBlocking) == hipSuccess) {
            bool ok1 = false, ok2 = false, ok3 = false;
            if (queues_independent(this, comm_st, stream, &ok1) == BDR_OK && queues_independent(this, comm_st, side, &ok2) == BDR_OK &&
                queues_independent(this, stream, comm_st, &ok3) == BDR_OK && ok1 && ok2 && ok3) comm_state = 1;
        }
    }
    if (comm_state != 1) return 0;
    segs[0] = ExchangeSeg{ar.w4, ar.total - ar.w4};
    segs[1] = ExchangeSeg{0, ar.w4};
    planes_stale(which);
    *comm = comm_st;
    xchg_epoch = sig_epoch;
    xchg_tracked = track_wait_pending && track_epoch == sig_epoch;
    hipLaunchKernelGGL(k_signal, dim3(1), dim3(64), 0, stream, sig, SIG_MAIN_END, xchg_epoch);
    return hipGetLastError() == hipSuccess ? 2 : 0;
}

int32_t DqnCnn::exchange_begin(int seg)
{
    const int flag = (seg == 0 && !xchg_tracked) ? SIG_SIDE : SIG_MAIN_END;
    return launch_gate(this, comm_st, flag, xchg_epoch, -1);
}

int32_t DqnCnn::exchange_end(int seg)
{
    hipLaunchKernelGGL(k_signal, dim3(1), dim3(64), 0, comm_st, sig, seg == 0 ? SIG_XFC : SIG_XCONV, xchg_epoch);
    BDR_HIP(hipGetLastError());
    if (seg == 0) xchg_pending_fc = true; else xchg_pending_conv = true;
    return BDR_OK;
}

int32_t DqnCnn::join_exchange(bool conv, bool fc)
{
    if (conv && xchg_pending_conv) { BDR_TRY(launch_gate(this, stream, SIG_XCONV, xchg_epoch, -1)); xchg_pending_conv = false; }
    if (fc && xchg_pending_fc) { BDR_TRY(launch_gate(this, stream, SIG_XFC, xchg_epoch, -1)); xchg_pending_fc = false; }
    return BDR_OK;
}

DqnCnn::~DqnCnn()
{
    (void)hipSetDevice(device);
    if (comm_st) { (void)hipStreamSynchronize(comm_st); (void)hipStreamDestroy(comm_st); }
    if (holds_gate_token) { DqnCnn* me = this; g_gate_owner.compare_exchange_strong(me, nullptr); holds_gate_token = false; }
    (void)hipStreamSynchronize(stream);
    if (side) (void)hipStreamSynchronize(side);
    free_batch_buffers(this);
    (void)hipFree(q); (void)hipFree(q_tgt); (void)hipFree(grad); (void)hipFree(m); (void)hipFree(v); (void)hipFree(vmax);
    (void)hipFree(loss); (void)hipFree(cpl[0]); (void)hipFree(cpl[1]);
    (void)hipFree(u_obs); (void)hipFree(u_next); (void)hipFree(u_act); (void)hipFree(u_rew); (void)hipFree(u_term);
    for (auto& e : ev_fork) if (e) (void)hipEventDestroy(e);
    if (ev_join) (void)hipEventDestroy(ev_join);
    if (gate_trace) {
        unsigned long long t[32] = {0};
        (void)hipMemcpy(t, gate_trace, sizeof t, hipMemcpyDeviceToHost);
        static const char* site[5] = {"side<-head", "side<-DxL1", "side<-DxC3", "-", "main<-side (join)"};
        for (int k = 0; k < 5; ++k)
            if (t[2 * k + 1]) fprintf(stderr, "gate %-18s mean wait %.2f us, longest %.1f us, over %llu gates\n", site[k], t[2 * k] / 100.0 / t[2 * k + 1], t[22 + k] / 100.0, t[2 * k + 1]);
        if (t[9]) fprintf(stderr, "the weight-gradient queue finished on average %.2f us before the dX queue reached the join\n", t[20] / 100.0 / (t[9] / 2.0));
        (void)hipFree(gate_trace);
    }
    if (sig) (void)hipFree(sig);
    (void)hipFree(applied_step); (void)hipFree(act_part); (void)hipFree(act_tickets);
    if (aux) { (void)hipStreamSynchronize(aux); stream_retire(aux); (void)hipStreamDestroy(aux); }
    if (side) { stream_retire(side); (void)hipStreamDestroy(side); }
}

int32_t DqnCnn::opt(bdr_replay* r) { return opt_inner(this, r); }

int32_t DqnCnn::apply_grads()
{
    BDR_TRY(adam_all(this));
    return after_updates(this);
}

static std::vector<NamedTensor> cnn_meta(int A, int ns);

int32_t DqnCnn::record(float* out, int cap, int* n)
{
    bdr_dqn_record rec{};
    BDR_TRY(fill_record(this, last_B, last_reward, &rec));
    std::vector<float> v = {rec.loss};
    if (rec.has_verbose) {
        v.insert(v.end(), {rec.pred_mean, rec.reward_mean, rec.tgt_mean, rec.tgt_minus_pred_mean});
        if (rec_opt) {
            std::vector<float> ref(ref_param_count(ar.A, ar.ns));
            BDR_TRY(get_params(0, ref.data(), ref.size()));
            param_stats(cnn_meta(ar.A, ar.ns), ref.data(), v);
            v.push_back(n_samples_act == 0 ? 0.f : (float)n_samples_best_act / (float)n_samples_act);
            n_samples_act = 0; n_samples_best_act = 0;
        }
    }
    for (size_t i = 0; i < v.size() && (int)i < cap; ++i) out[i] = v[i];
    *n = (int)std::min(v.size(), (size_t)cap);
    return BDR_OK;
}

void DqnCnn::record_keys(std::vector<std::string>& keys)
{
    keys = {"loss"};
    if (cfg.record_verbose_level >= 2) {
        keys.insert(keys.end(), {"pred_mean", "reward_mean", "tgt_mean", "tgt_minus_pred_mean"});
        param_stat_keys(cnn_meta(ar.A, ar.ns), keys);
        keys.push_back("ratio_best_act");
    }
}

uint64_t DqnCnn::param_count(int which) { return which == -1 ? (uint64_t)ar.A : ref_param_count(ar.A, ar.ns); }

int32_t DqnCnn::get_params(int which, float* out, uint64_t n)
{
    BDR_TRY(join_exchange(true, true));
    float* src = arena_ptr(this, which);
    BDR_REQUIRE(src, "which must be 0..4");
    BDR_REQUIRE(n == ref_param_count(ar.A, ar.ns), "parameter count mismatch (%llu vs %llu)", (unsigned long long)n,
                (unsigned long long)ref_param_count(ar.A, ar.ns));
    std::vector<float> in(ar.total);
    BDR_HIP(hipMemcpyAsync(in.data(), src, ar.total * 4, hipMemcpyDeviceToHost, stream));
    BDR_HIP(hipStreamSynchronize(stream));
    to_reference(ar, in.data(), out);
    return BDR_OK;
}

int32_t DqnCnn::set_params(int which, const float* inp, uint64_t n)
{
    BDR_TRY(join_exchange(true, true));
    float* dst = arena_ptr(this, which);
    BDR_REQUIRE(dst, "which must be 0..4");
    BDR_REQUIRE(n == ref_param_count(ar.A, ar.ns), "parameter count mismatch");
    std::vector<float> in(ar.total);
    to_internal(ar, inp, in.data());
    BDR_HIP(hipMemcpyAsync(dst, in.data(), ar.total * 4, hipMemcpyHostToDevice, stream));
    BDR_HIP(hipStreamSynchronize(stream));
    planes_stale(which);
    return BDR_OK;
}

float* DqnCnn::arena(int which, size_t* n)
{
    (void)join_exchange(true, true);
    planes_stale(which);
    if (n) *n = ar.total;
    return arena_ptr(this, which);
}

static std::vector<NamedTensor> cnn_meta(int A, int ns)
{
    return {{"c1.weight", {32, (uint64_t)ns, 8, 8}}, {"c1.bias", {32}}, {"c2.weight", {64, 32, 4, 4}}, {"c2.bias", {64}},
            {"c3.weight", {64, 64, 3, 3}}, {"c3.bias", {64}}, {"l1.weight", {512, 3136}}, {"l1.bias", {512}},
            {"l2.weight", {(uint64_t)A, 512}}, {"l2.bias", {(uint64_t)A}}};
}

int32_t DqnCnn::save(const char* dir)
{
    std::vector<float> ref(ref_param_count(ar.A, ar.ns));
    BDR_TRY(get_params(0, ref.data(), ref.size()));
    BDR_TRY(save_named(ckpt_save_path(this, dir, "qnet"), cnn_meta(ar.A, ar.ns), ref.data(), ref.size()));
    BDR_TRY(get_params(1, ref.data(), ref.size()));
    return save_named(ckpt_save_path(this, dir, "qnet_tgt"), cnn_meta(ar.A, ar.ns), ref.data(), ref.size());
}

int32_t DqnCnn::load(const char* dir)
{
    std::vector<float> ref(ref_param_count(ar.A, ar.ns));
    BDR_TRY(load_named(ckpt_load_path(this, dir, "qnet"), cnn_meta(ar.A, ar.ns), ref.data(), ref.size()));
    BDR_TRY(set_params(0, ref.data(), ref.size()));
    BDR_TRY(load_named(ckpt_load_path(this, dir, "qnet_tgt"), cnn_meta(ar.A, ar.ns), ref.data(), ref.size()));
    return set_params(1, ref.data(), ref.size());
}

namespace bdr {
int32_t dqn_cnn_create(const bdr_dqn_config* cfg, bdr_agent** out)
{
    BDR_REQUIRE(cfg->net.n_stack >= 1 && cfg->net.n_stack <= bdr::C1_MAX_STACK, "AtariCnnConfig::n_stack must be in [1, %d] (conv1's kernels are instantiated "
                "for these; the reference's examples use 4)", bdr::C1_MAX_STACK);
    BDR_REQUIRE(cfg->net.out_dim >= 1 && cfg->net.out_dim <= 64, "out_dim must be in [1,64]");
    DqnCnn* a = new DqnCnn();
    a->cfg = *cfg; a->device = cfg->device; a->train = cfg->train != 0;
    a->ar = make_arena(cfg->net.out_dim, cfg->net.n_stack);
    BDR_HIP(hipStreamCreateWithFlags(&a->stream, hipStreamNonBlocking));
    BDR_HIP(hipStreamCreateWithFlags(&a->side, hipStreamNonBlocking));
    for (auto& e : a->ev_fork) BDR_HIP(hipEventCreateWithFlags(&e, hipEventDisableTiming | hipEventDisableSystemFence));
    BDR_HIP(hipEventCreateWithFlags(&a->ev_join, hipEventDisableTiming | hipEventDisableSystemFence));
    if (const char* e = getenv("BDR_SCHED")) a->sched = std::max(0, std::min(3, atoi(e)));
    BDR_HIP(hipMalloc((void**)&a->sig, 16 * sizeof(unsigned)));
    BDR_HIP(hipMalloc((void**)&a->applied_step, 2 * sizeof(unsigned long long)));
    BDR_HIP(hipMemsetAsync(a->applied_step, 0, 2 * sizeof(unsigned long long), a->stream));
    BDR_HIP(hipMemsetAsync(a->sig, 0, 16 * sizeof(unsigned), a->stream));
    if (getenv("BDR_GATE_TRACE")) {
        BDR_HIP(hipMalloc((void**)&a->gate_trace, 32 * sizeof(unsigned long long)));
        BDR_HIP(hipMemsetAsync(a->gate_trace, 0, 32 * sizeof(unsigned long long), a->stream));
    }
    if (getenv("BDR_NO_OVERLAP")) a->sched = 0;
    if (const char* e = getenv("BDR_GATE_LIMIT_MS")) a->gate_limit = (unsigned long long)std::max(1, atoi(e)) * 100000ull;
    BDR_TRY(a->err_init());
    a->kev = getenv("BDR_NO_KEV") == nullptr;
    a->side_gather = getenv("BDR_NO_SIDE_GATHER") == nullptr;
    a->split_fwd = getenv("BDR_NO_SPLIT_FWD") == nullptr;
    a->conv_b3 = arith_is_split(cfg->arithmetic, "BDR_DQN_F32_EXACT");
    if (a->conv_b3) for (auto& pl : a->cpl) BDR_HIP(hipMalloc((void**)&pl, CPL_U16 * 2));
    { const char* e = getenv("BDR_TQ"); a->three_queues = !(e && e[0] == '0'); }
    float** arenas[5] = {&a->q, &a->q_tgt, &a->grad, &a->m, &a->v};
    for (auto p : arenas) {
        BDR_TRY(alloc_f(p, a->ar.total));
        BDR_HIP(hipMemsetAsync(*p, 0, a->ar.total * 4, a->stream));
    }
    a->amsgrad = cfg->opt_kind == BDR_OPT_ADAMW && cfg->amsgrad != 0;
    if (a->amsgrad) { BDR_TRY(alloc_f(&a->vmax, a->ar.total)); BDR_HIP(hipMemsetAsync(a->vmax, 0, a->ar.total * 4, a->stream)); }
    BDR_TRY(alloc_f(&a->loss, 4));
    std::vector<float> ref, in(a->ar.total);
    init_reference_params(a->ar.A, a->ar.ns, cfg->param_seed, ref);
    to_internal(a->ar, ref.data(), in.data());
    BDR_HIP(hipMemcpyAsync(a->q, in.data(), a->ar.total * 4, hipMemcpyHostToDevice, a->stream));
    BDR_HIP(hipMemcpyAsync(a->q_tgt, in.data(), a->ar.total * 4, hipMemcpyHostToDevice, a->stream));
    BDR_HIP(hipStreamSynchronize(a->stream));
    BDR_TRY(ensure_batch(a, (int)cfg->batch_size));
    BDR_HIP(hipStreamCreateWithFlags(&a->aux, hipStreamNonBlocking));
    if (a->sched == 3 && !getenv("BDR_SKIP_QUEUE_CHECK")) {
        bool ok1 = false, ok2 = false;
        BDR_TRY(queues_independent(a, a->side, a->stream, &ok1));
        BDR_TRY(queues_independent(a, a->stream, a->side, &ok2));
        BDR_TRY(queues_independent(a, a->aux, a->stream, &a->aux_gated));
        if (!(ok1 && ok2)) {
            fprintf(stderr, "border_amd: the agent's two streams share a hardware queue (GPU_MAX_HW_QUEUES?): serial backward schedule\n");
            a->sched = 0;
        }
    }
    *out = a;
    return BDR_OK;
}

int32_t dqn_cnn_update_on_batch(bdr_agent* base, uint64_t n, const void* obs, const int64_t* act, const void* next_obs,
                                const float* reward, const int8_t* term, const float* weight)
{
    DqnCnn* a = static_cast<DqnCnn*>(base);
    const size_t ob = (size_t)a->cfg.net.n_stack * 84 * 84;
    if (n > a->u_cap) {
        BDR_HIP(hipStreamSynchronize(a->stream));
        (void)hipFree(a->u_obs); (void)hipFree(a->u_next); (void)hipFree(a->u_act); (void)hipFree(a->u_rew); (void)hipFree(a->u_term);
        BDR_HIP(hipMalloc((void**)&a->u_obs, n * ob)); BDR_HIP(hipMalloc((void**)&a->u_next, n * ob));
        BDR_HIP(hipMalloc((void**)&a->u_act, n * 8)); BDR_HIP(hipMalloc((void**)&a->u_rew, n * 4));
        BDR_HIP(hipMalloc((void**)&a->u_term, round_up(n, 16)));
        a->u_cap = n;
    }
    BDR_HIP(hipMemcpyAsync(a->u_obs, obs, n * ob, hipMemcpyHostToDevice, a->stream));
    BDR_HIP(hipMemcpyAsync(a->u_next, next_obs, n * ob, hipMemcpyHostToDevice, a->stream));
    BDR_HIP(hipMemcpyAsync(a->u_act, act, n * 8, hipMemcpyHostToDevice, a->stream));
    BDR_HIP(hipMemcpyAsync(a->u_rew, reward, n * 4, hipMemcpyHostToDevice, a->stream));
    BDR_HIP(hipMemcpyAsync(a->u_term, term, n, hipMemcpyHostToDevice, a->stream));
    const float* wd = nullptr;
    if (weight) { BDR_TRY(a->td_buffer(n)); BDR_HIP(hipMemcpyAsync(a->w_stage, weight, n * 4, hipMemcpyHostToDevice, a->stream)); wd = a->w_stage; }
    const bool backward_only = a->defer_adam;
    if (a->amsgrad) a->defer_adam = true;
    const int32_t st = update_critic(a, (int)n, a->u_obs, a->u_next, a->u_act, 8, a->u_rew, a->u_term, wd, nullptr);
    a->defer_adam = backward_only;
    if (st == BDR_OK && !backward_only) {
        if (a->amsgrad) BDR_TRY(adam_all(a));
        BDR_TRY(after_updates(a));
    }
    BDR_TRY(st);
    BDR_HIP(hipStreamSynchronize(a->stream));
    return BDR_OK;
}

}

int32_t DqnCnn::grads_on_batch(uint64_t n, const void* obs, const int64_t* act, const void* next_obs, const float* reward, const int8_t* term)
{
    defer_adam = true;
    const int32_t st = bdr::dqn_cnn_update_on_batch(this, n, obs, act, next_obs, reward, term, nullptr);
    defer_adam = false;
    return st;
}

namespace bdr {
static int getenv_once_no_act_small()
{
    static const int v = getenv("BDR_NO_ACT_SMALL") ? 1 : 0;
    return v;
}

static int32_t act_small_forward(DqnCnn* a, const uint8_t* d, int n, float* q_out)
{
    const Arena& ar = a->ar;
    hipStream_t st = a->stream;
    BDR_TRY(a->join_exchange(true, true));
    if (!a->act_part) {
        BDR_HIP(hipMalloc((void**)&a->act_part, act_small_part_floats() * sizeof(float)));
        BDR_HIP(hipMalloc((void**)&a->act_tickets, ACT_SMALL_TICKETS * sizeof(unsigned)));
        BDR_HIP(hipMemsetAsync(a->act_tickets, 0, ACT_SMALL_TICKETS * sizeof(unsigned), st));
    }
    if (!a->rows_host) {
        BDR_HIP(hipHostMalloc((void**)&a->rows_host, (ROWS_PINNED_MAX_FLOATS + 16) * sizeof(float), hipHostMallocMapped));
        memset(a->rows_host, 0, (ROWS_PINNED_MAX_FLOATS + 16) * sizeof(float));
        BDR_HIP(hipHostGetDevicePointer((void**)&a->rows_dev, a->rows_host, 0));
    }
    {
        Conv1Args c{};
        c.M = n * 400; c.nz = 1; c.x[0] = d; c.w1[0] = a->q + ar.w1; c.bias[0] = a->q + ar.b1; c.out[0] = a->a1[0];
        if (ar.ns <= C1IMG_MAX_STACK) BDR_HIP(launch_conv1_bf16_img(ar.ns, 1, 16, dim3(n), st, c));
        else BDR_HIP(conv1_forward(ar.ns, n, st, c));
    }
    auto pad32 = [](int m) { return (m + 31) / 32 * 32; };
    ActLayerArgs l{};
    l.part = a->act_part; l.tickets = a->act_tickets; l.relu = 1;
    l.x = a->a1[0]; l.w = a->q + ar.w2; l.bias = a->q + ar.b2; l.out = a->a2[0]; l.M = n * 81; l.Mpad = pad32(l.M); l.N = 64; l.K = 512; l.KS = 4;
    BDR_HIP(launch_act_layer<2>(st, l));
    l.x = a->a2[0]; l.w = a->q + ar.w3; l.bias = a->q + ar.b3; l.out = a->a3[0]; l.M = n * 49; l.Mpad = pad32(l.M); l.N = 64; l.K = 576; l.KS = 3;
    BDR_HIP(launch_act_layer<3>(st, l));
    const unsigned seq = ++a->rows_seq;
    l.x = a->a3[0]; l.w = a->q + ar.w4; l.bias = a->q + ar.b4; l.out = a->h1[0]; l.M = n; l.Mpad = 32; l.N = 512; l.K = 3136; l.KS = 7;
    l.head = ActLayerArgs::Head{a->q + ar.w5, a->q + ar.b5, a->qv[0], n, ar.A, a->rows_dev + 16, reinterpret_cast<unsigned*>(a->rows_dev), seq,
                                (const unsigned*)a->dev_err, (int)bdr_agent::ERR_WORDS};
    BDR_HIP(launch_act_layer<0>(st, l));
    return a->rows_wait(seq, q_out, (size_t)n * ar.A);
}

int32_t dqn_cnn_qvalues(bdr_agent* base, uint64_t n, const void* obs, float* q_out)
{
    DqnCnn* a = static_cast<DqnCnn*>(base);
    BDR_TRY(ensure_batch(a, (int)n));
    const size_t ob = (size_t)a->cfg.net.n_stack * 84 * 84;
    const uint8_t* d = static_cast<const uint8_t*>(obs);
    const bool small = n <= (uint64_t)ACT_SMALL_MAX && !a->prof && getenv_once_no_act_small() == 0;
    if (small && !a->obs_rows_on_device) {
        BDR_TRY(a->host_rows_pinned(obs, n * ob, &d));
    } else if (!a->obs_in_place(ob)) {
        uint8_t* stage = nullptr;
        BDR_TRY(a->act_buffer(n * ob, (void**)&stage));
        BDR_TRY(a->stage_obs(stage, obs, ob, n, a->stream));
        d = stage;
    }
    if (small) {
        const int32_t st = act_small_forward(a, d, (int)n, q_out);
        a->slot_cursor = 0;
        return st;
    }
    NetInst inst[1] = {{d, a->q, 0}};
    int32_t st = forward(a, inst, 1, (int)n);
    if (st == BDR_OK) st = a->rows_to_host(a->qv[0], q_out, n * (size_t)a->ar.A);
    a->slot_cursor = 0;
    return st;
}

int32_t dqn_cnn_probe(bdr_agent* base, int32_t what, float* out, uint64_t n)
{
    DqnCnn* a = static_cast<DqnCnn*>(base);
    const float* src = nullptr;
    switch (what) {
        case 0: src = a->qv[0]; break;
        case 1: src = a->qv[1]; break;
        case 2: src = a->pred; break;
        case 3: src = a->tgt; break;
        case 4: src = a->loss; break;
        case 5: src = a->a1[0]; break;
        case 6: src = a->a2[0]; break;
        case 7: src = a->a3[0]; break;
        default: return fail(BDR_ERR_INVALID, "unknown probe %d", what);
    }
    BDR_REQUIRE(src, "nothing to probe yet (no update has run)");
    BDR_HIP(hipMemcpyAsync(out, src, n * 4, hipMemcpyDeviceToHost, a->stream));
    BDR_HIP(hipStreamSynchronize(a->stream));
    return BDR_OK;
}
}
```

Measured before the change: 5029.

## Overlap conv2/conv3 weight-grad and Adam tail with next step's forward

Splits the conv reduce+Adam tail into a conv1 segment on the main stream and a conv2/conv3 segment on the side stream. The side segment is gated on a start signal from the conv1 dW kernel and runs past the end of the step, joined lazily before the next conv2 forward or any host access. conv1 activations are double-buffered (a1_alt) so the next step's conv1 forward can run while the side work still reads the old buffer. This adds per-segment step-lag bookkeeping, a third applied-step slot and rollback logic, and it risks ordering bugs and contention between the two streams.

```diff
diff --git a/border_amd/csrc/conv1_dw_bf16.hpp b/border_amd/csrc/conv1_dw_bf16.hpp
--- a/border_amd/csrc/conv1_dw_bf16.hpp
+++ b/border_amd/csrc/conv1_dw_bf16.hpp
@@ -9,6 +9,8 @@
     float* part;
     size_t part_stride;
     int B;
+    unsigned* sig_flag;
+    unsigned sig_epoch;
 };
 
 constexpr int C1DW_LDM = 408;
@@ -81,6 +83,7 @@
 template <int NS>
 static __global__ __launch_bounds__(512) __attribute__((amdgpu_waves_per_eu(NS <= 4 ? C1DW_WAVES_PER_EU : 2, NS <= 4 ? C1DW_WAVES_PER_EU : 2))) void k_conv1_dw_bf16(Conv1DwArgs a)
 {
+    start_signal(a.sig_flag, a.sig_epoch);
     C1DW_TP(0);
     constexpr int TASKS = 4 * ((NS + 1) / 2), TPW = (TASKS + 7) / 8;
     extern __shared__ __attribute__((aligned(16))) uint8_t c1dw_lds[];
diff --git a/border_amd/csrc/dqn.hip b/border_amd/csrc/dqn.hip
--- a/border_amd/csrc/dqn.hip
+++ b/border_amd/csrc/dqn.hip
@@ -11,6 +11,7 @@
 #include "cnn_layers.hpp"
 #include "igemm_b3.hpp"
 #include "act_small.hpp"
+#include "dqn_rollback.hpp"
 
 using namespace bdr;
 
@@ -36,6 +37,9 @@
 #endif
 #ifndef BDR_TEAMS_DX_C2
 #define BDR_TEAMS_DX_C2 1
+#endif
+#ifndef BDR_TAIL_OVERLAP
+#define BDR_TAIL_OVERLAP 1
 #endif
 #ifndef BDR_DXC2_MERGED
 #define BDR_DXC2_MERGED 2
@@ -349,7 +353,11 @@
     uint64_t u_cap = 0;
     const float* last_reward = nullptr; int last_B = 0;
     uint64_t adam_step = 0, soft_update_counter = 0;
-    int64_t conv_step_lag = 0;
+    int64_t conv_lag[2] = {0, 0};
+    bool conv23_join_pending = false;
+    unsigned conv23_epoch = 0;
+    float* a1_alt = nullptr;
+    int32_t join_conv23();
     uint16_t* cpl[2] = {nullptr, nullptr};
     bool cpl_fresh[2] = {false, false}, cpl_escaped[2] = {false, false};
     bool conv_b3 = true;
@@ -372,7 +380,8 @@
     }
     int32_t after_sync() override
     {
-        if (!(xchg_pending_conv || xchg_pending_fc)) return BDR_OK;
+        if (!(xchg_pending_conv || xchg_pending_fc || conv23_join_pending)) return BDR_OK;
+        BDR_TRY(join_conv23());
         BDR_TRY(join_exchange(true, true));
         BDR_HIP(hipStreamSynchronize(stream));
         return BDR_OK;
@@ -405,13 +414,14 @@
     }
     (void)hipFree(a->dh1); (void)hipFree(a->dy3); (void)hipFree(a->dy2); (void)hipFree(a->dy1);
     (void)hipFree(a->dq); (void)hipFree(a->pred); (void)hipFree(a->tgt); (void)hipFree(a->loss_row);
-    (void)hipFree(a->part);
-    a->dh1 = a->dy3 = a->dy2 = a->dy1 = a->dq = a->pred = a->tgt = a->loss_row = a->part = nullptr;
+    (void)hipFree(a->part); (void)hipFree(a->a1_alt);
+    a->dh1 = a->dy3 = a->dy2 = a->dy1 = a->dq = a->pred = a->tgt = a->loss_row = a->part = a->a1_alt = nullptr;
 }
 
 int32_t ensure_batch(DqnCnn* a, int B)
 {
     if (B <= a->B) return BDR_OK;
+    BDR_TRY(a->join_conv23());
     BDR_HIP(hipStreamSynchronize(a->stream));
     free_batch_buffers(a);
     const int A = a->ar.A;
@@ -423,6 +433,7 @@
         BDR_TRY(alloc_f(&a->h1[z], (size_t)B * 512));
         BDR_TRY(alloc_f(&a->qv[z], (size_t)B * A));
     }
+    BDR_TRY(alloc_f(&a->a1_alt, (size_t)B * 400 * 32));
     BDR_TRY(alloc_f(&a->dh1, (size_t)B * 512));
     BDR_TRY(alloc_f(&a->dy3, (size_t)B * 49 * 64));
     BDR_TRY(alloc_f(&a->dy2, (size_t)B * 81 * 64));
@@ -446,9 +457,12 @@
     const unsigned* poison;
     int reduce_only;
     unsigned long long* applied; unsigned long long step;
+    unsigned long long* applied2;
+    int wg_base;
     uint16_t* cpl;
 };
 constexpr int SIG_HEAD = 0, SIG_DXL1 = 1, SIG_DXC3 = 2, SIG_SIDE = 3, SIG_GATHER = 4, SIG_TEST = 5, SIG_TEST_ERR = 6, SIG_ERR = 7, SIG_TGT = 8, SIG_TRACK = 9, SIG_MAIN_END = 10, SIG_XCONV = 11, SIG_XFC = 14;
+constexpr int SIG_DXC2 = 15, SIG_CONV23 = SIG_SIDE;
 __global__ __launch_bounds__(64) void k_gate(unsigned* sig, int which, unsigned epoch, unsigned long long* waited, int publish,
                                              unsigned long long limit = 1000000000ull , int err_slot = SIG_ERR,
                                              unsigned* dev_err = nullptr)
@@ -487,7 +501,7 @@
 __global__ __launch_bounds__(256) void k_reduce_adam(ConvReduceAdamArgs a)
 {
     const bool poisoned = a.reduce_only || (a.poison && *a.poison != 0);
-    if (a.applied && !poisoned && blockIdx.x == 0 && threadIdx.x == 0) *a.applied = a.step;
+    if (a.applied && !poisoned && blockIdx.x == 0 && threadIdx.x == 0) { *a.applied = a.step; if (a.applied2) *a.applied2 = a.step; }
     if ((int)blockIdx.x >= a.reduce_blocks) {
         if (poisoned) return;
         const size_t i = a.rest0_4 + (size_t)(blockIdx.x - a.reduce_blocks) * 256 + threadIdx.x;
@@ -506,10 +520,11 @@
         return;
     }
     __shared__ float red[8][32];
-    const int s_id = (int)blockIdx.x >= a.r.seg[2].wg0 ? 2 : ((int)blockIdx.x >= a.r.seg[1].wg0 ? 1 : 0);
+    const int bx = (int)blockIdx.x + a.wg_base;
+    const int s_id = bx >= a.r.seg[2].wg0 ? 2 : (bx >= a.r.seg[1].wg0 ? 1 : 0);
     const ReduceSeg& sg = a.r.seg[s_id];
     const int o = threadIdx.x & 31, grp = threadIdx.x >> 5;
-    const int i = ((int)blockIdx.x - sg.wg0) * 32 + o;
+    const int i = (bx - sg.wg0) * 32 + o;
     float s = 0.f;
     if (i < sg.n) {
         int c = grp;
@@ -558,6 +573,7 @@
         Bracket br(a, "fwd_conv1");
         BDR_HIP(conv1_forward(ar.ns, B, st, c));
     }
+    if (uses_q && st == a->stream) BDR_TRY(a->join_conv23());
     f.M = B * 81;
     for (int z = 0; z < nz; ++z) { f.x[z] = a->a1[inst[z].slot]; f.w[z] = inst[z].params + ar.w2; f.bias[z] = inst[z].params + ar.b2; f.out[z] = a->a2[inst[z].slot]; }
     bool b3 = a->conv_b3;
@@ -677,6 +693,7 @@
     a->last_reward = reward; a->last_B = B;
     const Arena& ar = a->ar;
     const bdr_dqn_config& c = a->cfg;
+    if (a->conv23_join_pending) std::swap(a->a1[0], a->a1_alt);
     NetInst inst[3] = {{obs, a->q, 0}, {next_obs, a->q_tgt, 1}, {next_obs, a->q, 2}};
 
     TdArgs t{};
@@ -715,6 +732,7 @@
     };
     const DwPlan pl = dw_plan(a->B, ar.ns);
     const bool defer = a->defer_adam;
+    const bool tail = gated && BDR_TAIL_OVERLAP != 0 && !defer;
     if (!defer) a->adam_step += 1;
     const AdamScalars adam_s = adam_scalars(c, std::max<uint64_t>(a->adam_step, 1));
 
@@ -778,9 +796,39 @@
     };
     auto c1_dw = [&]() -> int32_t {
         const int chunks = std::min(pl.chunks_c1, B);
-        Conv1DwArgs d{obs, a->dy1, a->part + pl.off_c1, pl.stride_c1, B};
+        Conv1DwArgs d{obs, a->dy1, a->part + pl.off_c1, pl.stride_c1, B, tail ? sigf(SIG_DXC2) : nullptr, epoch};
         Bracket br(a, "bwd_conv1_dw");
         BDR_HIP(launch_conv1_dw_bf16(ar.ns, dim3(chunks), a->stream, d));
+        return BDR_OK;
+    };
+
+    auto reduce_adam = [&](hipStream_t st, int lo, int hi) -> int32_t {
+        Reduce3Args r{};
+        const int Ms[3] = {B * 400, B * 81, B * 49};
+        const int plc[3] = {pl.chunks_c1, pl.chunks_c2, pl.chunks_c3};
+        const size_t offs[3] = {pl.off_c1, pl.off_c2, pl.off_c3}, strides[3] = {pl.stride_c1, pl.stride_c2, pl.stride_c3};
+        const size_t gw[3] = {ar.w1, ar.w2, ar.w3};
+        const int nw[3] = {(int)ar.n_w1(), 512 * 64, 576 * 64}, nb[3] = {32, 64, 64};
+        int wg = 0, wg0[4];
+        for (int k = 0; k < 3; ++k) {
+            const int nchunks = k == 0 ? std::min(plc[0], B) : std::min(plc[k], (Ms[k] + 31) / 32);
+            r.seg[k] = ReduceSeg{a->part + offs[k], strides[k], nchunks, a->grad + gw[k], nw[k] + nb[k], nw[k],
+                                 k == 0 ? INV255 : 1.0f, wg};
+            wg0[k] = wg;
+            wg += (nw[k] + nb[k] + 31) / 32;
+        }
+        wg0[3] = wg;
+        const int64_t lag = a->conv_lag[lo == 0 ? 0 : 1];
+        ConvReduceAdamArgs ra{};
+        ra.r = r; ra.p = a->q; ra.g = a->grad; ra.m = a->m; ra.v = a->v; ra.gbase = a->grad;
+        ra.rest0_4 = ra.n4 = ar.w4 / 4; ra.s = lag ? adam_scalars(c, (uint64_t)std::max<int64_t>((int64_t)a->adam_step - lag, 1)) : adam_s;
+        ra.applied = defer ? nullptr : a->applied_step + (lo == 0 ? 1 : 2); ra.step = (unsigned long long)((int64_t)a->adam_step - lag);
+        ra.applied2 = !defer && lo == 0 && hi == 3 ? a->applied_step + 2 : nullptr;
+        ra.wg_base = wg0[lo]; ra.reduce_blocks = wg0[hi] - wg0[lo]; ra.poison = a->sig + SIG_ERR; ra.reduce_only = defer ? 1 : 0;
+        ra.cpl = a->conv_b3 && !defer ? a->cpl[0] : nullptr;
+        hipLaunchKernelGGL(k_reduce_adam, dim3(ra.reduce_blocks), dim3(256), 0, st, ra);
+        BDR_HIP(hipGetLastError());
+        if (ra.cpl && hi > 1) a->cpl_fresh[0] = true;
         return BDR_OK;
     };
 
@@ -806,13 +854,26 @@
         BDR_TRY(head_bwd()); BDR_TRY(l1_dw());
         BDR_TRY(l1_dx());
         BDR_TRY(gate(sd, SIG_DXL1)); BDR_TRY(c3_dw()); BDR_TRY(adam_l1_l2());
-        hipLaunchKernelGGL(k_signal, dim3(1), dim3(64), 0, sd, a->sig, SIG_SIDE, epoch);
-        BDR_HIP(hipGetLastError());
+        if (!tail) {
+            hipLaunchKernelGGL(k_signal, dim3(1), dim3(64), 0, sd, a->sig, SIG_SIDE, epoch);
+            BDR_HIP(hipGetLastError());
+        }
         BDR_TRY(c3_dx());
         BDR_TRY(c2_dx());
-        { hipStream_t side = sd; sd = a->stream; BDR_TRY(c2_dw()); sd = side; }
-        BDR_TRY(c1_dw());
-        BDR_TRY(gate(a->stream, SIG_SIDE));
+        if (tail) {
+            BDR_TRY(c1_dw());
+            BDR_TRY(reduce_adam(a->stream, 0, 1));
+            BDR_TRY(gate(sd, SIG_DXC2));
+            BDR_TRY(c2_dw());
+            BDR_TRY(reduce_adam(sd, 1, 3));
+            hipLaunchKernelGGL(k_signal, dim3(1), dim3(64), 0, sd, a->sig, SIG_CONV23, epoch);
+            BDR_HIP(hipGetLastError());
+            a->conv23_join_pending = true; a->conv23_epoch = epoch;
+        } else {
+            { hipStream_t side = sd; sd = a->stream; BDR_TRY(c2_dw()); sd = side; }
+            BDR_TRY(c1_dw());
+            BDR_TRY(gate(a->stream, SIG_SIDE));
+        }
     } else if (sched == 2) {
         BDR_TRY(l1_dx());  BDR_TRY(head_bwd()); BDR_TRY(l1_dw());
         BDR_TRY(c3_dx());  BDR_TRY(adam_l1_l2()); BDR_TRY(c3_dw());
@@ -833,30 +894,10 @@
             BDR_HIP(hipStreamWaitEvent(a->stream, a->ev_join, 0));
         }
     }
-    {
-        Reduce3Args r{};
-        const int Ms[3] = {B * 400, B * 81, B * 49};
-        const int plc[3] = {pl.chunks_c1, pl.chunks_c2, pl.chunks_c3};
-        const size_t offs[3] = {pl.off_c1, pl.off_c2, pl.off_c3}, strides[3] = {pl.stride_c1, pl.stride_c2, pl.stride_c3};
-        const size_t gw[3] = {ar.w1, ar.w2, ar.w3};
-        const int nw[3] = {(int)ar.n_w1(), 512 * 64, 576 * 64}, nb[3] = {32, 64, 64};
-        int wg = 0;
-        for (int k = 0; k < 3; ++k) {
-            const int nchunks = k == 0 ? std::min(plc[0], B) : std::min(plc[k], (Ms[k] + 31) / 32);
-            r.seg[k] = ReduceSeg{a->part + offs[k], strides[k], nchunks, a->grad + gw[k], nw[k] + nb[k], nw[k],
-                                 k == 0 ? INV255 : 1.0f, wg};
-            wg += (nw[k] + nb[k] + 31) / 32;
-        }
-        ConvReduceAdamArgs ra{};
-        ra.r = r; ra.p = a->q; ra.g = a->grad; ra.m = a->m; ra.v = a->v; ra.gbase = a->grad;
-        ra.rest0_4 = ra.n4 = ar.w4 / 4; ra.s = a->conv_step_lag ? adam_scalars(c, (uint64_t)std::max<int64_t>((int64_t)a->adam_step - a->conv_step_lag, 1)) : adam_s;
-        ra.applied = defer ? nullptr : a->applied_step + 1; ra.step = (unsigned long long)((int64_t)a->adam_step - a->conv_step_lag);
-        ra.reduce_blocks = wg; ra.poison = a->sig + SIG_ERR; ra.reduce_only = defer ? 1 : 0;
-        ra.cpl = a->conv_b3 && !defer ? a->cpl[0] : nullptr;
+    if (!tail) {
         Bracket br(a, "reduce_adam");
-        hipLaunchKernelGGL(k_reduce_adam, dim3(wg), dim3(256), 0, a->stream, ra);
-        BDR_HIP(hipGetLastError());
-        if (ra.cpl) a->cpl_fresh[0] = true;
+        if (a->conv_lag[0] == a->conv_lag[1]) BDR_TRY(reduce_adam(a->stream, 0, 3));
+        else { BDR_TRY(reduce_adam(a->stream, 0, 1)); BDR_TRY(reduce_adam(a->stream, 1, 3)); }
     }
     return BDR_OK;
 }
@@ -865,6 +906,7 @@
 {
     const size_t n4 = a->ar.total / 4;
     const float tau = (float)a->cfg.tau, omt = (float)(1.0 - a->cfg.tau);
+    BDR_TRY(a->join_conv23());
     Bracket br(a, "track");
     a->planes_stale(1);
     hipLaunchKernelGGL(k_track, dim3((unsigned)((n4 + 255) / 256)), dim3(256), 0, a->stream, a->q_tgt, a->q, n4, tau, omt, (const unsigned*)(a->sig + SIG_ERR));
@@ -891,16 +933,17 @@
 
 int32_t adam_all(DqnCnn* a)
 {
+    BDR_TRY(a->join_conv23());
     a->adam_step += 1;
     a->planes_stale(0);
     Bracket br(a, "adam_all");
     const size_t n4 = a->ar.total / 4;
     const unsigned* poison = (const unsigned*)(a->sig + SIG_ERR);
-    struct Range { size_t off, n; uint64_t step; int slot; } rg[2] = {{0, a->ar.total, a->adam_step, 0}, {0, 0, 0, 1}};
+    struct Range { size_t off, n; uint64_t step; int slot; } rg[3] = {{0, a->ar.total, a->adam_step, 0}, {0, 0, 0, 1}, {0, 0, 0, 2}};
     int nr = 1;
-    if (a->conv_step_lag) {
-        const uint64_t cs = (uint64_t)std::max<int64_t>((int64_t)a->adam_step - a->conv_step_lag, 1);
-        rg[0] = Range{a->ar.w4, a->ar.total - a->ar.w4, a->adam_step, 0}; rg[1] = Range{0, a->ar.w4, cs, 1}; nr = 2;
+    if (a->conv_lag[0] || a->conv_lag[1]) {
+        const uint64_t c1s = (uint64_t)std::max<int64_t>((int64_t)a->adam_step - a->conv_lag[0], 1), c23s = (uint64_t)std::max<int64_t>((int64_t)a->adam_step - a->conv_lag[1], 1);
+        rg[0] = Range{a->ar.w4, a->ar.total - a->ar.w4, a->adam_step, 0}; rg[1] = Range{0, a->ar.w2, c1s, 1}; rg[2] = Range{a->ar.w2, a->ar.w4 - a->ar.w2, c23s, 2}; nr = 3;
     }
     for (int k = 0; k < nr; ++k) {
         const Range& g = rg[k];
@@ -911,8 +954,10 @@
         BDR_HIP(hipGetLastError());
     }
     if (nr == 1) {
-        hipLaunchKernelGGL(k_copy_word_unless, dim3(1), dim3(1), 0, a->stream, a->applied_step + 1, (const unsigned long long*)a->applied_step, poison);
-        BDR_HIP(hipGetLastError());
+        for (int k = 1; k <= 2; ++k) {
+            hipLaunchKernelGGL(k_copy_word_unless, dim3(1), dim3(1), 0, a->stream, a->applied_step + k, (const unsigned long long*)a->applied_step, poison);
+            BDR_HIP(hipGetLastError());
+        }
     }
     (void)n4;
     return BDR_OK;
@@ -976,6 +1021,7 @@
 
 int32_t fill_record(DqnCnn* a, int B, const float* reward_dev, bdr_dqn_record* rec)
 {
+    BDR_TRY(a->join_conv23());
     BDR_HIP(hipMemcpyAsync(&rec->loss, a->loss, 4, hipMemcpyDeviceToHost, a->stream));
     BDR_HIP(hipStreamSynchronize(a->stream));
     rec->has_verbose = 0;
@@ -1074,22 +1120,21 @@
     planes_stale(0); planes_stale(1);
     if (sig) (void)hipMemset(sig, 0, 16 * sizeof(unsigned));
     if (applied_step) {
-        unsigned long long applied[2] = {0, 0};
+        unsigned long long applied[3] = {0, 0, 0};
         if (hipMemcpy(applied, applied_step, sizeof applied, hipMemcpyDeviceToHost) == hipSuccess) {
-            const int64_t conv_now = (int64_t)adam_step - conv_step_lag;
-            if (applied[0] < adam_step || (int64_t)applied[1] < conv_now) {
-                const uint64_t skipped = adam_step - std::min<uint64_t>(applied[0], adam_step);
-                adam_step -= skipped;
-                conv_step_lag = (int64_t)adam_step - (int64_t)std::min<uint64_t>(applied[1], (uint64_t)std::max<int64_t>(conv_now, 0));
-                const uint64_t opts_back = std::min(n_opts, skipped / std::max<uint64_t>(1, cfg.n_updates_per_opt));
-                n_opts -= opts_back;
-                const uint64_t iv = std::max<uint64_t>(1, cfg.soft_update_interval);
-                soft_update_counter = (soft_update_counter + iv - opts_back % iv) % iv;
-                fprintf(stderr, "border_amd: %llu update(s) behind the failed gate were skipped on the device; the step counters were rolled back with them%s\n",
-                        (unsigned long long)skipped, conv_step_lag ? " (the conv segment is one optimizer step behind l1 / l2 and keeps its own step number)" : "");
+            const bdr::DqnRollback rb = bdr::dqn_rollback(applied, bdr::DqnStepCounters{adam_step, {conv_lag[0], conv_lag[1]}, n_opts, soft_update_counter},
+                                                          cfg.n_updates_per_opt, cfg.soft_update_interval);
+            if (rb.changed) {
+                adam_step = rb.c.adam_step; conv_lag[0] = rb.c.lag[0]; conv_lag[1] = rb.c.lag[1];
+                n_opts = rb.c.n_opts; soft_update_counter = rb.c.soft_update_counter;
+                fprintf(stderr, "border_amd: %llu update(s) behind the failed gate were skipped on the device; the step counters were rolled back with them", (unsigned long long)rb.skipped);
+                if (conv_lag[0] || conv_lag[1])
+                    fprintf(stderr, " (optimizer steps behind l1 / l2: conv1 %lld, conv2 + conv3 %lld - each segment keeps its own step number)", (long long)conv_lag[0], (long long)conv_lag[1]);
+                fprintf(stderr, "\n");
             }
         }
     }
+    conv23_join_pending = false;
     sig_epoch = 0; head_gate_enqueued = false;
     if (sched == 3) {
         fprintf(stderr, "border_amd: a cross-queue gate timed out; this agent continues with event ordering (schedule 1)\n");
@@ -1124,7 +1169,9 @@
 int32_t DqnCnn::exchange_begin(int seg)
 {
     const int flag = (seg == 0 && !xchg_tracked) ? SIG_SIDE : SIG_MAIN_END;
-    return launch_gate(this, comm_st, flag, xchg_epoch, -1);
+    BDR_TRY(launch_gate(this, comm_st, flag, xchg_epoch, -1));
+    if (flag == SIG_MAIN_END) BDR_TRY(launch_gate(this, comm_st, SIG_CONV23, xchg_epoch, -1));
+    return BDR_OK;
 }
 
 int32_t DqnCnn::exchange_end(int seg)
@@ -1133,6 +1180,13 @@
     BDR_HIP(hipGetLastError());
     if (seg == 0) xchg_pending_fc = true; else xchg_pending_conv = true;
     return BDR_OK;
+}
+
+int32_t DqnCnn::join_conv23()
+{
+    if (!conv23_join_pending) return BDR_OK;
+    conv23_join_pending = false;
+    return launch_gate(this, stream, SIG_CONV23, conv23_epoch, -1);
 }
 
 int32_t DqnCnn::join_exchange(bool conv, bool fc)
@@ -1149,6 +1203,7 @@
     if (holds_gate_token) { DqnCnn* me = this; g_gate_owner.compare_exchange_strong(me, nullptr); holds_gate_token = false; }
     (void)hipStreamSynchronize(stream);
     if (side) (void)hipStreamSynchronize(side);
+    conv23_join_pending = false;
     free_batch_buffers(this);
     (void)hipFree(q); (void)hipFree(q_tgt); (void)hipFree(grad); (void)hipFree(m); (void)hipFree(v); (void)hipFree(vmax);
     (void)hipFree(loss); (void)hipFree(cpl[0]); (void)hipFree(cpl[1]);
@@ -1214,6 +1269,7 @@
 
 int32_t DqnCnn::get_params(int which, float* out, uint64_t n)
 {
+    BDR_TRY(join_conv23());
     BDR_TRY(join_exchange(true, true));
     float* src = arena_ptr(this, which);
     BDR_REQUIRE(src, "which must be 0..4");
@@ -1228,6 +1284,7 @@
 
 int32_t DqnCnn::set_params(int which, const float* inp, uint64_t n)
 {
+    BDR_TRY(join_conv23());
     BDR_TRY(join_exchange(true, true));
     float* dst = arena_ptr(this, which);
     BDR_REQUIRE(dst, "which must be 0..4");
@@ -1242,6 +1299,7 @@
 
 float* DqnCnn::arena(int which, size_t* n)
 {
+    (void)join_conv23();
     (void)join_exchange(true, true);
     planes_stale(which);
     if (n) *n = ar.total;
@@ -1288,8 +1346,8 @@
     BDR_HIP(hipEventCreateWithFlags(&a->ev_join, hipEventDisableTiming | hipEventDisableSystemFence));
     if (const char* e = getenv("BDR_SCHED")) a->sched = std::max(0, std::min(3, atoi(e)));
     BDR_HIP(hipMalloc((void**)&a->sig, 16 * sizeof(unsigned)));
-    BDR_HIP(hipMalloc((void**)&a->applied_step, 2 * sizeof(unsigned long long)));
-    BDR_HIP(hipMemsetAsync(a->applied_step, 0, 2 * sizeof(unsigned long long), a->stream));
+    BDR_HIP(hipMalloc((void**)&a->applied_step, 3 * sizeof(unsigned long long)));
+    BDR_HIP(hipMemsetAsync(a->applied_step, 0, 3 * sizeof(unsigned long long), a->stream));
     BDR_HIP(hipMemsetAsync(a->sig, 0, 16 * sizeof(unsigned), a->stream));
     if (getenv("BDR_GATE_TRACE")) {
         BDR_HIP(hipMalloc((void**)&a->gate_trace, 32 * sizeof(unsigned long long)));
@@ -1339,6 +1397,7 @@
 {
     DqnCnn* a = static_cast<DqnCnn*>(base);
     const size_t ob = (size_t)a->cfg.net.n_stack * 84 * 84;
+    BDR_TRY(a->join_conv23());
     if (n > a->u_cap) {
         BDR_HIP(hipStreamSynchronize(a->stream));
         (void)hipFree(a->u_obs); (void)hipFree(a->u_next); (void)hipFree(a->u_act); (void)hipFree(a->u_rew); (void)hipFree(a->u_term);
@@ -1363,6 +1422,7 @@
         BDR_TRY(after_updates(a));
     }
     BDR_TRY(st);
+    BDR_TRY(a->join_conv23());
     BDR_HIP(hipStreamSynchronize(a->stream));
     return BDR_OK;
 }
@@ -1388,6 +1448,7 @@
 {
     const Arena& ar = a->ar;
     hipStream_t st = a->stream;
+    BDR_TRY(a->join_conv23());
     BDR_TRY(a->join_exchange(true, true));
     if (!a->act_part) {
         BDR_HIP(hipMalloc((void**)&a->act_part, act_small_part_floats() * sizeof(float)));
@@ -1423,6 +1484,7 @@
 int32_t dqn_cnn_qvalues(bdr_agent* base, uint64_t n, const void* obs, float* q_out)
 {
     DqnCnn* a = static_cast<DqnCnn*>(base);
+    BDR_TRY(a->join_conv23());
     BDR_TRY(ensure_batch(a, (int)n));
     const size_t ob = (size_t)a->cfg.net.n_stack * 84 * 84;
     const uint8_t* d = static_cast<const uint8_t*>(obs);
diff --git a/border_amd/csrc/dqn_rollback.hpp b/border_amd/csrc/dqn_rollback.hpp
--- /dev/null
+++ b/border_amd/csrc/dqn_rollback.hpp
@@ -0,0 +1,44 @@
+#pragma once
+#include <algorithm>
+#include <cstdint>
+
+namespace bdr {
+
+struct DqnStepCounters {
+    uint64_t adam_step;
+    int64_t lag[2];
+    uint64_t n_opts;
+    uint64_t soft_update_counter;
+};
+
+struct DqnRollback {
+    DqnStepCounters c;
+    uint64_t skipped;
+    bool changed;
+};
+
+inline DqnRollback dqn_rollback(const unsigned long long (&applied)[3], const DqnStepCounters& in, uint64_t n_updates_per_opt, uint64_t soft_update_interval)
+{
+    DqnRollback r{in, 0, false};
+    int64_t now[2];
+    bool behind = applied[0] < in.adam_step;
+    for (int k = 0; k < 2; ++k) {
+        now[k] = (int64_t)in.adam_step - in.lag[k];
+        behind = behind || (int64_t)applied[1 + k] < now[k];
+    }
+    if (!behind) return r;
+    r.changed = true;
+    r.skipped = in.adam_step - std::min<uint64_t>(applied[0], in.adam_step);
+    r.c.adam_step = in.adam_step - r.skipped;
+    for (int k = 0; k < 2; ++k) {
+        const uint64_t at = std::min<uint64_t>(applied[1 + k], (uint64_t)std::max<int64_t>(now[k], 0));
+        r.c.lag[k] = (int64_t)r.c.adam_step - (int64_t)at;
+    }
+    const uint64_t opts_back = std::min(in.n_opts, r.skipped / std::max<uint64_t>(1, n_updates_per_opt));
+    r.c.n_opts = in.n_opts - opts_back;
+    const uint64_t iv = std::max<uint64_t>(1, soft_update_interval);
+    r.c.soft_update_counter = (in.soft_update_counter + iv - opts_back % iv) % iv;
+    return r;
+}
+
+}
```

New measurement: 5270 (median of 6 runs). 4.8% higher.
